# zichunhao/lgn-autoencoder

Measured on AMD Instinct MI355X. Metric: jets/sec fwd+bwd, 30-particle maxdim=2 bs=512, higher is better.
Workload: dtype f64

## Files before the change

### include/lgn_amd.h

```cpp
#ifndef LGN_AMD_H
#define LGN_AMD_H

#include <stddef.h>
#include <stdint.h>

#ifdef __cplusplus
extern "C" {
#endif

#define LGN_AMD_ABI_VERSION 19

int lgn_abi_version(void);
const char* lgn_last_error(void);

int lgn_level_fwd_f64(int B, int N, int C, int CO, int decoder,
                      const double* s_in, const double* v_in, const double* p, const uint8_t* mask,
                      const double* ra, const double* rb, const double* rc,
                      const double* w0, const double* b0, const double* w1, const double* b1,
                      const double* wm0, const double* wm1,
                      double* ag0, double* ag1, double* s_out, double* v_out, void* stream);

int lgn_level_bwd_partial_rows(int B, int N, int decoder, int* rows_mix, int* rows_rad);
int lgn_level_rad_partial_len(int C, int decoder);
int lgn_level_jet_split(int B, int N);

int lgn_level_bwd_f64(int B, int N, int C, int CO, int decoder,
                      const double* s_in, const double* v_in, const double* p, const uint8_t* mask,
                      const double* ra, const double* rb, const double* rc,
                      const double* w0, const double* b0, const double* w1, const double* b1,
                      const double* wm0, const double* wm1, const double* ag0, const double* ag1,
                      const double* g_s_out, const double* g_v_out,
                      double* g_ag, double* g_s_in, double* g_v_in, double* g_p,
                      double* part_mix, double* part_rad, void* stream);

int lgn_cg_product_fwd_f64(int R, int N, int C, int D1, int D2, int DO, int mode, int nnz, const int* row_ptr, const int* col,
                           const double* coef, const double* x1, const double* x2, double* out, void* stream);
int lgn_cg_product_bwd_f64(int R, int N, int C, int D1, int D2, int DO, int mode, int nnz, const int* row_ptr, const int* col,
                           const double* coef, const double* x1, const double* x2, const double* g_out, double* g_x1, double* g_x2,
                           void* stream);

int lgn_reduce_partials_f64(const double* part, int rows, int n, double* out, int accumulate, void* stream);

int lgn_radial_finalize_f64(const double* tot, int C, const double* ra, const double* rb, const double* rc,
                            const double* w0, const double* w1,
                            double* g_a, double* g_b, double* g_c,
                            double* g_w0, double* g_b0, double* g_w1, double* g_b1, void* stream);

#define LGN_ACT_LEAKYRELU 0
#define LGN_ACT_RELU 1
#define LGN_ACT_ELU 2
#define LGN_ACT_SIGMOID 3
#define LGN_ACT_LOGSIGMOID 4
#define LGN_ACT_ATAN 5
#define LGN_ACT_COUNT 6
int lgn_cgmlp_fwd_f64(int M, int C, int H, int nlin, int activation, const double* const* w, const double* const* b,
                      const double* s_in, double* s_out, void* stream);
int lgn_cgmlp_partial_rows(int M, int H);
int lgn_cgmlp_bwd_f64(int M, int C, int H, int nlin, int activation, const double* const* w, const double* const* b,
                      const double* s_in, const double* g_out, double* g_in, double* part, int psize, void* stream);

int lgn_mixreps_fwd_f64(int rows, int Cin, int Cout, int d, const double* w, const double* x, double* y, void* stream);
int lgn_mixreps_partial_rows(int rows);
int lgn_mixreps_bwd_f64(int rows, int Cin, int Cout, int d, const double* w, const double* x, const double* g_y,
                        double* g_x, double* part, void* stream);

int lgn_moments_fwd_f64(int B, int N, int C, int Q, int decoder, const double* X, const double* p, const uint8_t* mask,
                        const double* ra, const double* rb, const double* rc, const double* w0, const double* b0,
                        const double* w1, const double* b1, double* U, void* stream);
long long lgn_moments_scratch_doubles(int B, int N, int C, int decoder);
int lgn_moments_bwd_f64(int B, int N, int C, int Q, int decoder, const double* X, const double* p, const uint8_t* mask,
                        const double* ra, const double* rb, const double* rc, const double* w0, const double* b0,
                        const double* w1, const double* b1, const double* gU, double* gX, double* g_p,
                        double* part_rad, double* scratch, void* stream);

typedef struct lgn_local_tables {
  int n_rows, n_out, n_w;
  int n_terms, n_u, n_x;
  int n_units, static_kind;
  const int *row_ptr, *t_type, *t_a, *t_b;
  const double* t_coef;
  const int *out_dim, *out_nblk, *out_row0, *out_q0, *out_w0;
  const int *u_ptr, *u_row;
  const double* u_coef;
  const int *x_ptr, *x_row, *x_other;
  const double* x_coef;
  int h_out_w0[8];
} lgn_local_tables;

int lgn_local_fwd_f64(int nodes, int C, int CO, int Q, int Qout, const lgn_local_tables* t, const double* X, const double* U,
                      const double* wcat, double* out, void* stream);
int lgn_local_partial_rows(int nodes);
int lgn_local_bwd_f64(int nodes, int C, int CO, int Q, int Qout, const lgn_local_tables* t, const double* X, const double* U,
                      const double* wcat, const double* g_out, double* gU, double* gX, double* part, void* stream);

long long lgn_local_static_packed_doubles(int kind, int C, int CO);
int lgn_local_bwd_static_f64(int kind, int nodes, int C, int CO, const double* XT, const double* UT, const double* wcat,
                             const int* w0, double* wpacked, const double* goT, double* gUT, double* gXT, double* part,
                             double* gpacked, double* g_wcat, void* stream);
int lgn_local_fwd_static_f64(int kind, int nodes, int C, int CO, const double* XT, const double* UT, const double* wcat,
                             const int* w0, double* wpacked, double* outT, double* s_copy, int q_s, void* stream);

typedef struct lgn_net_desc {
  int B, N;
  int n_levels;
  int enc_channels[5];
  int dec_channels[5];
  int tau_s, tau_v;
  int mlp_hidden_mul;
  int mlp_nlin;
  int tau_v_in;
  const lgn_local_tables* enc_tables[4];
  const lgn_local_tables* dec_tables[4];
  int enc_Q[5], enc_qs[5], enc_qv[5];
  int dec_Q[5], dec_qs[5], dec_qv[5];
  int flags;
  int activation;
  int n_in_scalars;
  int latent_pool;
  int dec_N;
  int get_real;
  double jet_loss_scale;
} lgn_net_desc;
#define LGN_REAL_SUM 0
#define LGN_REAL_REAL 1
#define LGN_REAL_IMAG 2
#define LGN_REAL_MEAN 3
#define LGN_REAL_NORM 4
#define LGN_LOSS_CHAMFER 0
#define LGN_LOSS_MSE 1
#define LGN_LOSS_HUNGARIAN 2
typedef struct lgn_loss_desc {
  int kind;
  int abs_coord;
  int polar_coord;
  double scale;
} lgn_loss_desc;
#define LGN_POOL_MIN 0
#define LGN_POOL_MAX 1
#define LGN_POOL_MEAN 2
#define LGN_POOL_MIX 3
#define LGN_POOL(n, avg, o0, o1, o2, o3) ((n) | ((avg) << 3) | ((o0) << 4) | ((o1) << 6) | ((o2) << 8) | ((o3) << 10))
#define LGN_NET_NO_STATIC 1
#define LGN_NET_DEC_PAIRWISE 2
#define LGN_NET_LEVEL_V2 4
#define LGN_NET_MLP_V1 8
#define LGN_NET_MOMENTS_V1 16
#define LGN_NET_BWD_ORDERED 64
#define LGN_NET_DEC_UNFUSED 256
#define LGN_NET_MOMENTS_SPLIT 512
#define LGN_NET_MLP_BWD1 1024
#define LGN_NET_SPLIT_TAIL 128

#define LGN_LDS_LIMIT (160 * 1024)
long long lgn_encoder_end_lds_bytes(int N, int C0, int K, int CL, int Ts, int Tv, int pool);
long long lgn_decoder_end_lds_bytes(int N, int C0, int Tin, int CL);
long long lgn_junction_lds_bytes(int N, int CL, int Ts, int Tv, int pool, int C0);

int lgn_step_param_slots(const lgn_net_desc* d, int decoder);
long long lgn_step_workspace_doubles(const lgn_net_desc* d);
int lgn_step_fwd_bwd_f64(const lgn_net_desc* d, const double* params, double* grads, long long n_params,
                         const int64_t* enc_off, const int64_t* dec_off, const double* p4, const double* target,
                         const uint8_t* mask, const double* in_scalars, double* workspace, long long workspace_doubles,
                         double* recon, double* loss_part, const lgn_loss_desc* loss, int* assignment ,
                         int* status , void* stream);
#define LGN_FINALIZE_SCRATCH 2048
int lgn_step_finalize_f64(double* params, double* grads, long long n_params, const double* loss_part, int n_loss,
                          double l1_lambda, double* adam_m, double* adam_v, long long* step_dev,
                          double lr, double beta1, double beta2, double eps, int do_adam, double* loss_out, void* stream);
int lgn_step_train_f64(const lgn_net_desc* d, double* params, double* grads, long long n_params, const int64_t* enc_off,
                       const int64_t* dec_off, const double* p4, const double* target, const uint8_t* mask, const double* in_scalars,
                       double* workspace, long long workspace_doubles, double* recon, double* loss_part, int n_loss, double l1_lambda,
                       double* adam_m, double* adam_v, long long* step_dev, double lr, double beta1, double beta2, double eps,
                       int do_adam, double* loss_out, const lgn_loss_desc* loss, int* assignment ,
                       int* status , void* stream);

#define LGN_OPT_ADAM 0
#define LGN_OPT_RMSPROP 1
typedef struct {
  int kind;
  double l1_lambda, l2_lambda, lr, eps;
  double beta1, beta2;
  double alpha, momentum;
} lgn_optim_desc;
#define LGN_FINALIZE_OPT_SCRATCH 4096
int lgn_step_finalize_opt_f64(double* params, double* grads, long long n_params, const double* loss_part, int n_loss,
                              const lgn_optim_desc* opt, double* state_m, double* state_v, long long* step_dev, int do_step,
                              double* loss_out, void* stream);
int lgn_step_train_opt_f64(const lgn_net_desc* d, double* params, double* grads, long long n_params, const int64_t* enc_off,
                           const int64_t* dec_off, const double* p4, const double* target, const uint8_t* mask,
                           const double* in_scalars, double* workspace, long long workspace_doubles, double* recon,
                           double* loss_part, int n_loss, const lgn_optim_desc* opt, double* state_m, double* state_v,
                           long long* step_dev, int do_step, double* loss_out, const lgn_loss_desc* loss,
                           int* assignment , int* status , void* stream);

long long lgn_eval_workspace_doubles(const lgn_net_desc* d);
int lgn_step_eval_f64(const lgn_net_desc* d, const double* params, const int64_t* enc_off, const int64_t* dec_off,
                      const double* p4_scaled, const double* p4_target, const uint8_t* mask, const double* in_scalars,
                      double* workspace, long long workspace_doubles, double* recon_real, double* lat_s ,
                      double* lat_v , double* loss_part, double* loss_out, const lgn_loss_desc* loss,
                      int* assignment , int* status , void* stream);

long long lgn_net_workspace_doubles(const lgn_net_desc* d, int decoder, int which);
int lgn_encoder_fwd_f64(const lgn_net_desc* d, const double* params, const int64_t* off, const double* p4, const uint8_t* mask,
                        const double* in_scalars, double* act, long long act_doubles, double* lat_s, double* lat_v, void* stream);
int lgn_encoder_bwd_f64(const lgn_net_desc* d, const double* params, double* grads, long long n_params, const int64_t* off,
                        const double* p4, const uint8_t* mask, const double* in_scalars, const double* act, long long act_doubles,
                        const double* g_lat_s, const double* g_lat_v, double* scratch, long long scratch_doubles, void* stream);
int lgn_decoder_fwd_f64(const lgn_net_desc* d, const double* params, const int64_t* off, const double* lat_v, double* act,
                        long long act_doubles, double* recon, void* stream);
int lgn_decoder_bwd_f64(const lgn_net_desc* d, const double* params, double* grads, long long n_params, const int64_t* off,
                        const double* lat_v, const double* act, long long act_doubles, const double* g_recon, double* g_lat_v,
                        double* scratch, long long scratch_doubles, void* stream);

int lgn_chamfer_f64(int B, int N, int M, const double* x, const double* y, int jet_features, double* loss_part, double* gx, double* gy,
                    void* stream);

#define LGN_ANOMALY_NMAX 192
#define LGN_ANOMALY_NSCORES 21
#define LGN_ANOMALY_ALL 0x1FFFFF
#define LGN_ANOMALY_HUNGARIAN 0x403E0
#define LGN_ANOMALY_NO_HUNGARIAN (LGN_ANOMALY_ALL & ~LGN_ANOMALY_HUNGARIAN)
int lgn_anomaly_scores_f64(const double* recons, const double* target, const double* recons_n, const double* target_n, int B, int N,
                           int score_mask, double* scores, int* col4row , int* status, void* stream);

#define LGN_ROC_TILE 2048
#define LGN_ROC_MAX_COLS 65535
#define LGN_ROC_NONFINITE 1
#define LGN_ROC_SINGLE_CLASS 2
#define LGN_ROC_BAD_LABEL 4
#define LGN_ROC_NAN 8
long long lgn_roc_workspace_bytes(long long M, int K);
int lgn_roc_auc_f64(const double* scores, long long M, int ld, int K, const double* labels, double* fpr, double* tpr,
                    double* thresholds, int* length, double* auc, int* flipped, int* status, void* workspace,
                    long long workspace_bytes, void* stream);

#define LGN_EMD_NMAX 191
#define LGN_EMD_INVALID 1
#define LGN_EMD_EMPTY 2
#define LGN_EMD_ITER 4
#define LGN_EMD_INFEASIBLE 8
long long lgn_emd_workspace_bytes(int B, int N);
long long lgn_emd_lds_bytes(int N);
int lgn_emd_f64(const double* ev0, const double* ev1, int B, int n, int m, double R, double* emd, double* flow ,
                double* dual0 , double* dual1 , int* status, void* work, long long work_bytes, void* stream);
int lgn_emd_relative_f64(const double* recons, const double* target, int B, int N, double* emd, int* status, void* work,
                         long long work_bytes, void* stream);
int lgn_emd_debug_max_augmentations(int* out, int reset);

int lgn_linear_sum_assignment_f64(const double* cost, int B, int n, int* col4row, int* status, void* stream);

int lgn_recon_analysis_f64(const double* target, const double* recons, int B, int N, int abs_coord, int find_match,
                           double* part_polar , double* part_polarrel , double* jet_cart, double* jet_polar,
                           double* jet_rel_err, uint8_t* jet_keep, double* rel_err , int* col4row ,
                           uint8_t* is_padded, int* status, void* stream);

int lgn_match_rel_err_f64(const double* target3, const double* recons3, const double* target_polar, const double* recons_polar,
                          const double* target_polarrel, const double* recons_polarrel, int B, int N, double* rel_err,
                          int* col4row , uint8_t* is_padded, int* status, void* stream);

#define LGN_HIST_MAX_EDGES 1025
#define LGN_HIST_MAX_COLS 16
int lgn_histogram_f64(const double* x, long long rows, int ld, int cols, const double* edges, const int* n_edges , int max_edges,
                      const uint8_t* keep , const double* weights , long long* counts, double* wcounts,
                      int max_bins, void* stream);

#define LGN_STATS_TILE 2048
#define LGN_STATS_MAX_COLS 16
#define LGN_STATS_EMPTY 1
#define LGN_STATS_NONFINITE 2
#define LGN_STAT_MEDIAN 0
#define LGN_STAT_IQR 1
#define LGN_STAT_FIRST_QUARTILE 2
#define LGN_STAT_THIRD_QUARTILE 3
#define LGN_STAT_IDR 4
#define LGN_STAT_MAD 5
#define LGN_STAT_MEAN 6
#define LGN_STAT_MAX 7
#define LGN_STAT_MIN 8
#define LGN_STAT_ABS_MIN 9
#define LGN_STAT_STD_DEV 10
#define LGN_STAT_SKEW 11
#define LGN_STAT_KURTOSIS 12
#define LGN_STAT_FWHM 13
#define LGN_STAT_ABS_MEAN 14
#define LGN_STAT_ABS_MEAN_WITHIN_IQR 15
#define LGN_STAT_ABS_MEAN_WITHIN_IDR 16
#define LGN_STAT_Q10 17
#define LGN_STAT_Q90 18
#define LGN_STATS_COUNT 19
long long lgn_column_stats_workspace_bytes(long long rows, int cols);
int lgn_column_stats_f64(const double* x, long long rows, int ld, int cols, const uint8_t* mask , int mask_keep,
                         double alpha, int num_edges, double* stats ,
                         double* edges , long long* kept ,
                         int* status , void* workspace, long long workspace_bytes, void* stream);

int lgn_hist_fwhm_f64(const long long* counts, int max_bins, const double* edges, int max_edges, const int* n_edges , int cols,
                      double* fwhm , void* stream);

#define LGN_JET_IMAGE_MAX_NPIX 64
#define LGN_JET_IMAGE_PARTS 512
long long lgn_jet_images_workspace_bytes(int B, int npix);
int lgn_jet_images_f64(const double* jets, const double* frame_jets , int B, int N, int mode, int npix, double maxR,
                       int first_n, double* images , double* average, void* workspace, long long workspace_bytes,
                       void* stream);

#define LGN_EQUI_TILE 256
#define LGN_EQUI_MAX_PARTS 64
int lgn_transform_jets_f64(const double* p4, const double* R, const int* perm , const double* scalars , int T,
                           int B, int N, int K, double* out, double* scalars_out , void* stream);
long long lgn_rep_deviation_workspace_bytes(int parts, int T, int B, const int* N , const int* C ,
                                            const int* d );
int lgn_rep_deviation_f64(int parts, int T, int B, const double* const* a , const double* const* b ,
                          const double* const* D , const int* N , const int* C , const int* d ,
                          const int* perm , double* stats , void* workspace, long long workspace_bytes,
                          void* stream);

int lgn_hungarian_mse_f64(int B, int N, const double* x, const double* y, int kind, int abs_coord, int polar_coord, double scale,
                          double* loss_part, double* gx, int* assignment , int* status ,
                          void* stream);
long long lgn_assign_loss_lds_bytes(int N, int C);

#define LGN_NORM_NONE 0
#define LGN_NORM_COMPONENT_MAX 1
#define LGN_NORM_OVERALL_MAX 2
#define LGN_NORM_JET_E 3
int lgn_stage_batch_f64(const double* p4, const uint8_t* labels , const double* scalars , int B, int B_pad, int N,
                        int method, double scale, int jet_features, int K, double* p4_in, double* target, uint8_t* mask,
                        double* in_scalars , double* factor, void* stream);
int lgn_denormalize_f64(const double* x0, const double* x1 , const double* factor, int B, int N, double* out0,
                        double* out1 , void* stream);

#define LGN_EPOCH_MAX_COLLECT 4
#define LGN_EPOCH_BAD_INDEX 1
int lgn_stage_gather_f64(const double* p4, const uint8_t* labels , const double* scalars , long long M,
                         const int* index, long long count, const long long* cursor, int B_pad, int N, int method, double scale,
                         int jet_features, int K, double* p4_in, double* target, uint8_t* mask, double* in_scalars ,
                         double* factor, int* status, void* stream);
int lgn_epoch_collect_f64(const double* loss, double* epoch, long long* cursor, long long count, int B, int n,
                          const double* const* src , double* const* dst , const int* row_doubles , void* stream);
int lgn_epoch_reset(long long* cursor, double* epoch, int* status, void* stream);

#ifdef __cplusplus
}
#endif
#endif
```

### lgn-autoencoder_amd/csrc/api_common.cpp

```cpp
#include <stdarg.h>
#include <stdlib.h>

#include "level.hpp"
#include "../../include/lgn_amd.h"

namespace lgn {
static thread_local char g_err[512] = "";
void set_error(const char* fmt, ...) {
  va_list ap;
  va_start(ap, fmt);
  vsnprintf(g_err, sizeof(g_err), fmt, ap);
  va_end(ap);
}
int level_flags_from_env() {
  auto on = [](const char* name) { const char* e = getenv(name); return e && e[0] == '1'; };
  return (on("LGN_AMD_DEC_PAIRWISE") ? LVL_DEC_PAIRWISE : 0) | (on("LGN_AMD_LEVEL_V2") ? LVL_LEVEL_V2 : 0) |
         (on("LGN_AMD_MOMENTS_V1") ? LVL_MOMENTS_V1 : 0) | (on("LGN_AMD_MLP_V1") ? LVL_MLP_V1 : 0) | (on("LGN_AMD_BWD_ORDERED") ? LVL_BWD_ORDERED : 0) |
         (on("LGN_AMD_MOMENTS_SPLIT") ? LVL_MOMENTS_SPLIT : 0) | (on("LGN_AMD_MLP_BWD1") ? LVL_MLP_BWD1 : 0);
}
static_assert(LVL_DEC_PAIRWISE == LGN_NET_DEC_PAIRWISE && LVL_LEVEL_V2 == LGN_NET_LEVEL_V2 && LVL_MOMENTS_V1 == LGN_NET_MOMENTS_V1 &&
                  LVL_MLP_V1 == LGN_NET_MLP_V1 && LVL_MLP_BWD1 == LGN_NET_MLP_BWD1 &&
                  LVL_BWD_ORDERED == LGN_NET_BWD_ORDERED && LVL_MOMENTS_SPLIT == LGN_NET_MOMENTS_SPLIT, "LVL_* and LGN_NET_* are the same bits");
}

extern "C" {
const char* lgn_last_error(void) { return lgn::g_err; }
int lgn_abi_version(void) { return LGN_AMD_ABI_VERSION; }
}
```

### lgn-autoencoder_amd/csrc/level.hpp

```cpp
#pragma once
#include "common.hpp"

namespace lgn {

constexpr int LVL_DEC_PAIRWISE = 2;
constexpr int LVL_LEVEL_V2 = 4;
constexpr int LVL_MLP_V1 = 8;
constexpr int LVL_MOMENTS_V1 = 16;
constexpr int LVL_MLP_BWD1 = 1024;
constexpr int LVL_MOMENTS_SPLIT = 512;
constexpr int LVL_BWD_ORDERED = 64;
int level_flags_from_env();

template <typename T>
struct LevelArgs {
  int B, N, C, CO;
  const T* s_in;
  const T* v_in;
  const T* p;
  const uint8_t* mask;
  const T *ra, *rb, *rc, *w0, *b0, *w1, *b1;
  const T *wm0, *wm1;
  T* ag0;
  T* ag1;
  T* s_out;
  T* v_out;
  const T* in_w0 = nullptr;
  const T* in_w1 = nullptr;
  T* in_s = nullptr;
  T* in_v = nullptr;
  T* z1 = nullptr;
  size_t z1n = 0;
  T* z2 = nullptr;
  size_t z2n = 0;
  const T* loss_wo1 = nullptr;
  const T* loss_target = nullptr;
  T loss_scale = T(1);
  int loss_real = 0;
  T loss_jscale = T(0);
  T* loss_recon = nullptr;
  T* loss_part = nullptr;
  T* loss_gv = nullptr;
  T* loss_wpart = nullptr;
  int flags = 0;
};

template <typename T>
struct LevelBwdArgs {
  int B, N, C, CO;
  const T *s_in, *v_in, *p;
  const uint8_t* mask;
  const T *ra, *rb, *rc, *w0, *b0, *w1, *b1;
  const T *wm0, *wm1;
  const T *ag0, *ag1;
  const T* g_s_out;
  const T* g_v_out;
  T* g_ag;
  T* g_s_in;
  T* g_v_in;
  T* g_p;
  T* part_mix;
  T* part_rad;
  T* part_in0 = nullptr;
  int flags = 0;
};

__host__ __device__ constexpr int node_stride(int C) { return 10 * C + 4; }

__host__ __device__ constexpr int rad_partial_size(int C, bool dec) {
  return dec ? 2 * C : (2 * 4 * C * NB + 8 * C);
}

inline int level_jet_split(int B, int N) {
  const int groups = (N + 3) / 4;
  int s = 1;
  while (s * 2 <= groups && B * s * 2 <= 512) s *= 2;
  return s;
}

}
```

### lgn-autoencoder_amd/csrc/mlp_chain.hip

```cpp
#include "ops.hpp"

namespace lgn {

typedef double v4d __attribute__((ext_vector_type(4)));
namespace { LGN_STAMP_DECL }
#ifdef LGN_STAMPS
#define DSTAMP(i) do { if (threadIdx.x == 256 && blockIdx.x == 0) g_stamps[i] = clock64(); } while (0)
#else
#define DSTAMP(i) do { } while (0)
#endif
LGN_STAMP_READER(lgn_debug_stamps_mlp_chain)

namespace chain {

__host__ __device__ constexpr int stride2mod4(int x) { return x + ((6 - (x & 3)) & 3); }

__device__ __forceinline__ void lds_barrier() {
  __builtin_amdgcn_sched_barrier(0);
  __builtin_amdgcn_fence(__ATOMIC_RELEASE, "workgroup", "local");
  __builtin_amdgcn_s_barrier();
  __builtin_amdgcn_fence(__ATOMIC_ACQUIRE, "workgroup", "local");
  __builtin_amdgcn_sched_barrier(0);
}
template <int N, int P, class LoadF, class MmaF, class SideF>
__device__ __forceinline__ void mfma_stream(LoadF load, MmaF mma, SideF side) {
  double q[N];
#pragma unroll
  for (int i = 0; i < (P < N ? P : N); ++i) q[i] = load(i);
  __builtin_amdgcn_sched_barrier(0);
#pragma unroll
  for (int i = 0; i < N; ++i) {
    if (i + P < N) q[i + P] = load(i + P);
    mma(i, q[i]);
    side(i);
    __builtin_amdgcn_sched_barrier(0);
  }
}
constexpr int LOOKAHEAD = 9;
template <int N, int T, class F>
__device__ __forceinline__ void deal(int i, F piece) {
  const int j0 = (i * T + N - 1) / N, j1 = ((i + 1) * T + N - 1) / N;
#pragma unroll
  for (int j = j0; j < j1; ++j) piece(j);
}
__device__ __forceinline__ void pin(double& x) { asm volatile("" : "+v"(x)); }

#ifndef LGN_DBG_NOSTAGE
#define LGN_DBG_NOSTAGE 0
#endif
#ifndef LGN_DBG_NOACT
#define LGN_DBG_NOACT 0
#endif
template <bool GEN>
__device__ __forceinline__ double act_t(double x, int act) {
  if (LGN_DBG_NOACT) return x;
  if constexpr (GEN) return act_apply(x, act);
  else return fmax(x, 0.01 * x);
}
template <int H_, int D_, int NST_ = 256>
struct Geo {
  static constexpr int H = H_, D = D_, NH = 6;
  static constexpr int NST = NST_;
  static constexpr int NT = (H + 15) / 16, HP = 16 * NT;
  static constexpr int KSH = H / 4;
  static constexpr int KS0 = (D + 3) / 4;
  static constexpr int S = stride2mod4(HP + 1);
  static constexpr int WSIZE = HP * S;
  static constexpr int SR = NST == 256 ? 66 : 18;
  static constexpr int TSIZE = HP * SR;
  static constexpr int NREG = (HP * 2 * KSH + NST - 1) / NST;
  static_assert(H % 4 == 0 && D <= 16 && D <= H && H <= 96, "chain kernels: H = 12 .. 96 (multiple of 4; the backward: H <= 48), 2C <= 16");
  static constexpr size_t fwd_bytes() { return sizeof(double) * 2 * WSIZE; }
  static constexpr size_t bwd_bytes() { return sizeof(double) * (2 * WSIZE + 4 * TSIZE + (NST == 256 ? 2 * 1024 : 0)); }
  static constexpr int off_w(int l) { return l == 0 ? 0 : (H * D + H) + (l - 1) * (H * H + H); }
  static constexpr int hout(int l) { return l == NH ? D : H; }
  static constexpr int hin(int l) { return l == 0 ? D : H; }
  static constexpr int off_b(int l) { return off_w(l) + hout(l) * hin(l); }
  static constexpr int psize() { return off_b(NH) + D; }
};

template <class G, int L>
struct Img {
  static constexpr int HO = G::hout(L), HI = G::hin(L);
  static constexpr int RP = L == G::NH ? 16 : G::HP;
  static constexpr int CP = L == 0 ? 4 * G::KS0 : 4 * G::KSH;
  static constexpr int CP2 = CP / 2;
  static constexpr int NP = (RP * CP2 + G::NST - 1) / G::NST;
  static_assert(NP <= G::NREG && HI % 2 == 0, "staging registers; rows of an even number of doubles");
};
typedef double v2d __attribute__((ext_vector_type(2)));
template <class G>
struct WRegs {
  v2d v[G::NREG];
  double b;
};
template <class G, int L>
__device__ __forceinline__ void issue_piece(const MlpArgs<double>& a, WRegs<G>& wr, int tid, int j) {
  using I = Img<G, L>;
  if (j < I::NP) {
    const int e = tid + G::NST * j, o = e / I::CP2, k = 2 * (e - o * I::CP2);
    const bool ok = o < I::HO && k < I::HI;
    const v2d x = *reinterpret_cast<const v2d*>(a.w[L] + (ok ? o * I::HI + k : 0));
    wr.v[j] = ok ? x : v2d{0.0, 0.0};
  } else if (j == I::NP) {
    const double bb = a.b[L][tid < I::HO ? tid : 0];
    wr.b = tid < I::HO ? bb : 0.0;
  }
}
template <class G, int L>
__device__ __forceinline__ void commit_piece(double* Wl, const WRegs<G>& wr, int tid, int j) {
  using I = Img<G, L>;
  if (j < I::NP) {
    const int e = tid + G::NST * j, o = e / I::CP2, k = 2 * (e - o * I::CP2);
    if (I::RP * I::CP2 % G::NST == 0 || e < I::RP * I::CP2) *reinterpret_cast<v2d*>(Wl + o * G::S + k) = wr.v[j];
  } else if (j == I::NP) {
    if (tid < I::RP) Wl[tid * G::S + G::HP] = wr.b;
  }
}
template <class G, int L>
__device__ __forceinline__ void issue_image(const MlpArgs<double>& a, WRegs<G>& wr, int tid) {
  using I = Img<G, L>;
#pragma unroll
  for (int i = 0; i < I::NP + 1; ++i) issue_piece<G, L>(a, wr, tid, i);
}
template <class G, int L>
__device__ __forceinline__ void commit_image(double* Wl, const WRegs<G>& wr, int tid) {
  using I = Img<G, L>;
#pragma unroll
  for (int i = 0; i < I::NP + 1; ++i) commit_piece<G, L>(Wl, wr, tid, i);
}
template <class G, bool BWD>
__host__ __device__ constexpr int seq(int q) { return BWD && q > G::NH ? 2 * G::NH - q : q; }
template <class G>
constexpr int stage_pieces() { return 2 * (G::NREG + 1); }
template <class G, bool BWD, int Q>
__device__ __forceinline__ void stage_piece(const MlpArgs<double>& a, double* Wl, WRegs<G>& wrA, WRegs<G>& wrB, int tid, int j) {
  constexpr int LAST = BWD ? 2 * G::NH : G::NH, n1 = Q + 1, n3 = Q + 3;
  WRegs<G>& wr = (n1 & 1) ? wrB : wrA;
  if (j <= G::NREG) {
    if constexpr (n1 <= LAST) commit_piece<G, seq<G, BWD>(n1 <= LAST ? n1 : 0)>(Wl + (n1 & 1) * G::WSIZE, wr, tid, j);
  } else {
    if constexpr (n3 <= LAST) issue_piece<G, seq<G, BWD>(n3 <= LAST ? n3 : 0)>(a, wr, tid, j - G::NREG - 1);
  }
}
template <class G, bool BWD>
__device__ __forceinline__ void stage_prologue(const MlpArgs<double>& a, double* Wl, WRegs<G>& wrA, WRegs<G>& wrB, int tid) {
  issue_image<G, 0>(a, wrA, tid);
  issue_image<G, 1>(a, wrB, tid);
  commit_image<G, 0>(Wl, wrA, tid);
  issue_image<G, 2>(a, wrA, tid);
}

template <class G, int KS, int NTI, bool GEN, int DBG = 0, class ExtF>
__device__ __forceinline__ void layer_fwd(const double* Wc, const v4d (&hin)[NTI], v4d (&hout)[G::NT], int c, int g, int act, ExtF ext) {
  constexpr int S = G::S, NT = G::NT;
  const double* wa = Wc + c * S + g;
  const double* wbias = Wc + g * S + G::HP;
  v4d acc[NT];
#pragma unroll
  for (int r = 0; r < 4; ++r) acc[0][r] = wbias[4 * r * S];
  if (DBG) STAMP(30);
  mfma_stream<KS * NT, LOOKAHEAD>(
      [&](int i) { return wa[16 * (i / KS) * S + 4 * (i % KS)]; },
      [&](int i, double av) {
        const int t = i / KS, ks = i % KS;
        acc[t] = __builtin_amdgcn_mfma_f64_16x16x4f64(av, hin[ks >> 2][ks & 3], acc[t], 0, 0, 0);
      },
      [&](int i) {
        const int t = i / KS, ks = i % KS;
        if (ks == 0 && t + 1 < NT) {
#pragma unroll
          for (int r = 0; r < 4; ++r) acc[t + 1 < NT ? t + 1 : 0][r] = wbias[(16 * (t + 1) + 4 * r) * S];
        }
        constexpr int k1 = KS > 6 ? 5 : KS > 1 ? 1 : 0, k2 = KS > 6 ? 6 : KS > 2 ? 2 : k1;
#pragma unroll
        for (int r = 0; r < 4; ++r)
          if (t > 0 && ks == (r < 2 ? k1 : k2)) {
            double y = act_t<GEN>(acc[t > 0 ? t - 1 : 0][r], act);
            pin(y);
            hout[t > 0 ? t - 1 : 0][r] = y;
          }
        ext(i);
        if (DBG && (i == 0 || i == 1 || i == 2 || i == 11 || i == 12 || i == 23 || i == 34 || i == 35)) STAMP(31 + i);
      });
  if (DBG) STAMP(28);
#pragma unroll
  for (int r = 0; r < 4; ++r) hout[NT - 1][r] = act_t<GEN>(acc[NT - 1][r], act);
  if (DBG) { double z_ = hout[NT - 1][3]; pin(z_); hout[NT - 1][3] = z_; STAMP(29); }
}
template <class G>
__device__ __forceinline__ v4d layer_out(const double* Wc, const v4d (&hin)[G::NT], int c, int g) {
  constexpr int S = G::S;
  const double* wa = Wc + c * S + g;
  v4d acc;
#pragma unroll
  for (int r = 0; r < 4; ++r) acc[r] = Wc[(4 * r + g) * S + G::HP];
  mfma_stream<G::KSH, LOOKAHEAD>([&](int ks) { return wa[4 * ks]; },
                                 [&](int ks, double av) { acc = __builtin_amdgcn_mfma_f64_16x16x4f64(av, hin[ks >> 2][ks & 3], acc, 0, 0, 0); },
                                 [&](int) {});
  return acc;
}
template <class G, int KS, int NTO, int NTG, class FinF, class ExtF>
__device__ __forceinline__ void layer_bwd(const double* Wc, const v4d (&gpre)[NTG], v4d (&gin)[NTO], int c, int g, FinF fin, ExtF ext) {
  constexpr int S = G::S;
  const double* wa = Wc + g * S + c;
#pragma unroll
  for (int u = 0; u < NTO; ++u) gin[u] = v4d{0, 0, 0, 0};
  mfma_stream<KS * NTO, LOOKAHEAD>(
      [&](int i) { return wa[4 * (i % KS) * S + 16 * (i / KS)]; },
      [&](int i, double av) {
        const int u = i / KS, ks = i % KS;
        gin[u] = __builtin_amdgcn_mfma_f64_16x16x4f64(av, gpre[ks >> 2][ks & 3], gin[u], 0, 0, 0);
      },
      [&](int i) {
        const int u = i / KS, ks = i % KS;
        constexpr int k1 = KS > 6 ? 5 : KS > 1 ? 1 : 0, k2 = KS > 6 ? 6 : KS > 2 ? 2 : k1;
#pragma unroll
        for (int r = 0; r < 4; ++r)
          if (u > 0 && ks == (r < 2 ? k1 : k2)) fin(u > 0 ? u - 1 : 0, r);
        ext(i);
      });
}

template <class G>
__device__ __forceinline__ double* saved_ptr(const MlpArgs<double>& a, int wave, int lane) {
  return a.h_saved + ((size_t)blockIdx.x * 4 + wave) * (G::NH * G::NT * 256) + lane * 4;
}
template <class G>
constexpr int saved_pieces() { return 2 * G::NT; }
template <class G, int NTI>
__device__ __forceinline__ void save_piece(double* hs, int l, const v4d (&h)[NTI], int j) {
  const v2d v = {h[j >> 1][2 * (j & 1)], h[j >> 1][2 * (j & 1) + 1]};
  __builtin_nontemporal_store(v, reinterpret_cast<v2d*>(hs + (l * G::NT + (j >> 1)) * 256 + 2 * (j & 1)));
}
template <class G>
__device__ __forceinline__ void load_piece(const double* hs, int l, v4d (&h)[G::NT], int j) {
  const v2d v = __builtin_nontemporal_load(reinterpret_cast<const v2d*>(hs + (l * G::NT + (j >> 1)) * 256 + 2 * (j & 1)));
  h[j >> 1][2 * (j & 1)] = v[0];
  h[j >> 1][2 * (j & 1) + 1] = v[1];
}

template <class G>
__device__ __forceinline__ void load_x(const MlpArgs<double>& a, int row, int g, v4d (&xb)[1]) {
  const bool rok = row < a.M;
#pragma unroll
  for (int r = 0; r < 4; ++r) {
    const int f = 4 * r + g;
    const bool ok = r < G::KS0 && rok && f < G::D;
    const double x = a.s_in[ok ? (size_t)(f & 1) * a.M * a.C + (size_t)row * a.C + (f >> 1) : 0];
    xb[0][r] = ok ? x : 0.0;
  }
}

template <int H, int D, bool GEN, bool SAVE, bool TWO = false>
__global__ __launch_bounds__(TWO ? 512 : 256) void mlp_chain_fwd_kernel(MlpArgs<double> a) {
  using G = Geo<H, D>;
  const int tid = threadIdx.x, lane = tid & 63, wave = __builtin_amdgcn_readfirstlane(tid >> 6);
  const int c = lane & 15, g = lane >> 4;
  const int row = blockIdx.x * 64 + wave * 16 + c;
  extern __shared__ __align__(16) unsigned char smem_raw[];
  double* Wl = reinterpret_cast<double*>(smem_raw);
  WRegs<G> wrA, wrB;
  STAMP(0);
  STAMP_LIFE_BEGIN();
  if constexpr (TWO) {
    if (wave >= 4) {
      const int st = tid - 256;
      stage_prologue<G, false>(a, Wl, wrA, wrB, st);
      lds_barrier();
#define LGN_STAGE_STEP(Q)                                                                                            \
  _Pragma("unroll") for (int j = 0; j < stage_pieces<G>(); ++j) stage_piece<G, false, Q>(a, Wl, wrA, wrB, st, j);    \
  lds_barrier();
      LGN_STAGE_STEP(0) LGN_STAGE_STEP(1) LGN_STAGE_STEP(2) LGN_STAGE_STEP(3) LGN_STAGE_STEP(4) LGN_STAGE_STEP(5)
#undef LGN_STAGE_STEP
      return;
    }
  }
  v4d xb[1];
  load_x<G>(a, row, g, xb);
  if constexpr (!TWO) stage_prologue<G, false>(a, Wl, wrA, wrB, tid);
  lds_barrier();
  STAMP(1);
  v4d h0[G::NT], h1[G::NT];
  double* hs = SAVE ? saved_ptr<G>(a, wave, lane) : nullptr;
#define LGN_CHAIN_STEP(Q, HIN, HOUT, KS, NTI)                                                                        \
  layer_fwd<G, KS, NTI, GEN, (Q == 3)>(Wl + (Q & 1) * G::WSIZE, HIN, HOUT, c, g, a.act, [&](int i) {               \
    if (!TWO && !LGN_DBG_NOSTAGE) deal<KS * G::NT, stage_pieces<G>()>(i, [&](int j) { stage_piece<G, false, Q>(a, Wl, wrA, wrB, tid, j); });      \
    if (SAVE && Q > 0) deal<KS * G::NT, 2 * NTI>(i, [&](int j) { save_piece<G>(hs, Q - 1, HIN, j); });              \
  });                                                                                                                \
  lds_barrier();                                                                                                     \
  STAMP(2 + Q);
  LGN_CHAIN_STEP(0, xb, h0, G::KS0, 1)
  LGN_CHAIN_STEP(1, h0, h1, G::KSH, G::NT)
  LGN_CHAIN_STEP(2, h1, h0, G::KSH, G::NT)
  LGN_CHAIN_STEP(3, h0, h1, G::KSH, G::NT)
  LGN_CHAIN_STEP(4, h1, h0, G::KSH, G::NT)
  LGN_CHAIN_STEP(5, h0, h1, G::KSH, G::NT)
#undef LGN_CHAIN_STEP
  if (SAVE) {
#pragma unroll
    for (int j = 0; j < saved_pieces<G>(); ++j) save_piece<G>(hs, G::NH - 1, h1, j);
  }
  const v4d y = layer_out<G>(Wl + (G::NH & 1) * G::WSIZE, h1, c, g);
#pragma unroll
  for (int r = 0; r < 4; ++r) {
    const int o = 4 * r + g;
    if (o < D && row < a.M) a.s_out[mlp_out_index(a, o & 1, row, o >> 1)] = y[r];
  }
  STAMP(8);
  STAMP_LIFE_END();
}

template <class G, int NTI>
__device__ __forceinline__ void publish_piece(double* T, const v4d (&v)[NTI], int wave, int c, int g, int j) {
  T[(4 * j + g) * G::SR + 16 * wave + c] = v[j >> 2][j & 3];
}
template <class G, int L, int NU, class SideF>
__device__ __forceinline__ void dw_unit(const double* Gt, const double* Xt, double* part, int t, int u0, int c, int g, SideF side) {
  constexpr int SR = G::SR, HO = G::hout(L), HI = G::hin(L), N = 16 * NU, P = 6;
  const double* ga = Gt + (16 * t + c) * SR + g;
  const double* xb = Xt + (16 * u0 + c) * SR + g;
  double* pW = part + G::off_w(L);
  v4d acc[NU];
#pragma unroll
  for (int u = 0; u < NU; ++u) acc[u] = v4d{0, 0, 0, 0};
  double dbs = 0.0, qa[16], qx[N];
  auto load = [&](int i) {
    qx[i] = xb[16 * (i >> 4) * SR + 4 * (i & 15)];
    if (i < 16) qa[i] = ga[4 * i];
  };
  auto store = [&](int u, int r) {
    const int o = 16 * t + 4 * r + g, k = 16 * (u0 + u) + c;
    if (o < HO && k < HI) __builtin_nontemporal_store(acc[u][r], &pW[o * HI + k]);
  };
#pragma unroll
  for (int i = 0; i < P; ++i) load(i);
  __builtin_amdgcn_sched_barrier(0);
#pragma unroll
  for (int i = 0; i < N; ++i) {
    const int u = i >> 4, sk = i & 15;
    if (i + P < N) load(i + P);
    acc[u] = __builtin_amdgcn_mfma_f64_16x16x4f64(qa[sk], qx[i], acc[u], 0, 0, 0);
    if (u > 0 && sk >= 1 && sk <= 4) store(u > 0 ? u - 1 : 0, sk - 1);
    side(i);
    __builtin_amdgcn_sched_barrier(0);
  }
#pragma unroll
  for (int r = 0; r < 4; ++r) store(NU - 1, r);
  if (u0 == 0) {
    double d4[4] = {0.0, 0.0, 0.0, 0.0};
#pragma unroll
    for (int sk = 0; sk < 16; ++sk) d4[sk & 3] += qa[sk];
    dbs = (d4[0] + d4[1]) + (d4[2] + d4[3]);
    dbs += shfl_xor(dbs, 16);
    dbs += shfl_xor(dbs, 32);
    if (g == 0 && 16 * t + c < HO) __builtin_nontemporal_store(dbs, &part[G::off_b(L) + 16 * t + c]);
  }
}
template <class G, int L, class SideF>
__device__ __forceinline__ bool dw_layer(const double* Gt, const double* Xt, double* part, int wave, int c, int g, SideF side) {
  if (L == G::NH) {
    if (wave < G::NT) { dw_unit<G, L, 1>(Gt, Xt, part, 0, wave, c, g, side); return true; }
  } else if (L == 0) {
    if (wave < G::NT) { dw_unit<G, L, 1>(Gt, Xt, part, wave, 0, c, g, side); return true; }
  } else {
    const int t = (wave + L) & 3;
    if (t < G::NT) { dw_unit<G, L, G::NT>(Gt, Xt, part, t, 0, c, g, side); return true; }
  }
  return false;
}

template <int H, int D, bool GEN, bool SAVE>
__global__ __launch_bounds__(256) void mlp_chain_bwd_kernel(MlpArgs<double> a) {
  using G = Geo<H, D>;
  constexpr int NT = G::NT, NH = G::NH;
  const int tid = threadIdx.x, lane = tid & 63, wave = __builtin_amdgcn_readfirstlane(tid >> 6);
  const int c = lane & 15, g = lane >> 4;
  const int row = blockIdx.x * 64 + wave * 16 + c;
  extern __shared__ __align__(16) unsigned char smem_raw[];
  double* Wl = reinterpret_cast<double*>(smem_raw);
  double* Gt = Wl + 2 * G::WSIZE;
  double* Xt = Gt + 2 * G::TSIZE;
  double* part = a.part + (size_t)blockIdx.x * a.psize;
  WRegs<G> wrA, wrB;
  STAMP(10);
  v4d xb[1];
  load_x<G>(a, row, g, xb);
  v4d gout[1];
#pragma unroll
  for (int r = 0; r < 4; ++r) {
    const int o = 4 * r + g;
    const bool ok = o < D && row < a.M;
    const double x = a.g_out[ok ? mlp_out_index(a, o & 1, row, o >> 1) : 0];
    gout[0][r] = ok ? x : 0.0;
  }
  v4d h[NH][NT];
  const double* hs = SAVE ? saved_ptr<G>(a, wave, lane) : nullptr;
  if constexpr (SAVE) {
    issue_image<G, NH>(a, wrA, tid);
    issue_image<G, NH - 1>(a, wrB, tid);
#pragma unroll
    for (int j = 0; j < saved_pieces<G>(); ++j) load_piece<G>(hs, NH - 1, h[NH - 1], j);
#pragma unroll
    for (int j = 0; j < saved_pieces<G>(); ++j) load_piece<G>(hs, NH - 2, h[NH - 2], j);
    commit_image<G, NH>(Wl, wrA, tid);
    issue_image<G, NH - 2>(a, wrA, tid);
    lds_barrier();
    STAMP(11);
  } else {
    stage_prologue<G, true>(a, Wl, wrA, wrB, tid);
    lds_barrier();
    STAMP(11);
#define LGN_CHAIN_STEP(Q, HIN, KS, NTI)                                                                              \
  layer_fwd<G, KS, NTI, GEN>(Wl + (Q & 1) * G::WSIZE, HIN, h[Q], c, g, a.act, [&](int i) {                          \
    deal<KS * NT, stage_pieces<G>()>(i, [&](int j) { stage_piece<G, true, Q>(a, Wl, wrA, wrB, tid, j); });          \
  });                                                                                                                \
  lds_barrier();                                                                                                     \
  STAMP(12 + Q);
    LGN_CHAIN_STEP(0, xb, G::KS0, 1)
    LGN_CHAIN_STEP(1, h[0], G::KSH, NT)
    LGN_CHAIN_STEP(2, h[1], G::KSH, NT)
    LGN_CHAIN_STEP(3, h[2], G::KSH, NT)
    LGN_CHAIN_STEP(4, h[3], G::KSH, NT)
    LGN_CHAIN_STEP(5, h[4], G::KSH, NT)
#undef LGN_CHAIN_STEP
  }
  v4d gpA[NT], gpB[NT], gin[NT];
  {
    constexpr int NI = G::KS0 * NT, NSV = SAVE && NH >= 3 ? saved_pieces<G>() : 0, NPC = 4 + 4 * NT + stage_pieces<G>() + NSV;
    auto fin = [&](int u, int r) {
      double y = gin[u][r] * act_slope_t<GEN>(h[NH - 1][u][r], a.act);
      pin(y);
      gpA[u][r] = y;
    };
    layer_bwd<G, G::KS0, NT, 1>(Wl + 0 * G::WSIZE, gout, gin, c, g, fin, [&](int i) {
      deal<NI, NPC>(i, [&](int j) {
        if (j < 4) publish_piece<G, 1>(Gt, gout, wave, c, g, j);
        else if (j < 4 + 4 * NT) publish_piece<G, NT>(Xt, h[NH - 1], wave, c, g, j - 4);
        else if (j < 4 + 4 * NT + stage_pieces<G>()) stage_piece<G, true, NH>(a, Wl, wrA, wrB, tid, j - 4 - 4 * NT);
        else if constexpr (NSV > 0) load_piece<G>(hs, NH - 3, h[NH >= 3 ? NH - 3 : 0], j - 4 - 4 * NT - stage_pieces<G>());
      });
    });
#pragma unroll
    for (int r = 0; r < 4; ++r) fin(NT - 1, r);
    lds_barrier();
    STAMP(18);
  }
#define LGN_CHAIN_BSTEP(L, GP, GN)                                                                                   \
  {                                                                                                                  \
    constexpr int q_ = 2 * NH - (L), NI = G::KSH * NT, NSV = SAVE && (L) >= 3 ? saved_pieces<G>() : 0,               \
                  NPC = 8 * NT + stage_pieces<G>() + NSV;                                                            \
    auto fin = [&](int u, int r) {                                                                                   \
      double y = gin[u][r] * act_slope_t<GEN>(h[(L) - 1][u][r], a.act);                                              \
      pin(y);                                                                                                        \
      GN[u][r] = y;                                                                                                  \
    };                                                                                                               \
    layer_bwd<G, G::KSH, NT, NT>(Wl + (q_ & 1) * G::WSIZE, GP, gin, c, g, fin, [&](int i) {                          \
      deal<NI, NPC>(i, [&](int j) {                                                                                  \
        if (j < 4 * NT) publish_piece<G, NT>(Gt + ((L) & 1) * G::TSIZE, GP, wave, c, g, j);                          \
        else if (j < 8 * NT) publish_piece<G, NT>(Xt + ((L) & 1) * G::TSIZE, h[(L) - 1], wave, c, g, j - 4 * NT);    \
        else if (j < 8 * NT + stage_pieces<G>()) stage_piece<G, true, q_>(a, Wl, wrA, wrB, tid, j - 8 * NT);         \
        else if constexpr (NSV > 0) load_piece<G>(hs, (L) - 3, h[(L) >= 3 ? (L) - 3 : 0], j - 8 * NT - stage_pieces<G>()); \
      });                                                                                                            \
    });                                                                                                              \
    auto tail = [&](int i) {                                                                                         \
      if (i == 1) { fin(NT - 1, 0); fin(NT - 1, 1); }                                                                \
      if (i == 2) { fin(NT - 1, 2); fin(NT - 1, 3); }                                                                \
    };                                                                                                               \
    if (!dw_layer<G, (L) + 1>(Gt + (((L) + 1) & 1) * G::TSIZE, Xt + (((L) + 1) & 1) * G::TSIZE, part, wave, c, g, tail)) {   \
      tail(1);                                                                                                       \
      tail(2);                                                                                                       \
    }                                                                                                                \
    lds_barrier();                                                                                                   \
    STAMP(12 + q_);                                                                                                  \
  }
  LGN_CHAIN_BSTEP(5, gpA, gpB)
  LGN_CHAIN_BSTEP(4, gpB, gpA)
  LGN_CHAIN_BSTEP(3, gpA, gpB)
  LGN_CHAIN_BSTEP(2, gpB, gpA)
  LGN_CHAIN_BSTEP(1, gpA, gpB)
#undef LGN_CHAIN_BSTEP
  {
    v4d gx[1];
    layer_bwd<G, G::KSH, 1, NT>(Wl + 0 * G::WSIZE, gpB, gx, c, g, [&](int, int) {}, [&](int i) {
      deal<G::KSH, 4 * NT + 4>(i, [&](int j) {
        if (j < 4 * NT) publish_piece<G, NT>(Gt, gpB, wave, c, g, j);
        else publish_piece<G, 1>(Xt, xb, wave, c, g, j - 4 * NT);
      });
    });
    auto tail = [&](int i) {
      if (i >= 1 && i <= 4) {
        const int f = 4 * (i - 1) + g;
        if (f < D && row < a.M) a.g_in[mlp_out_index(a, f & 1, row, f >> 1)] = gx[0][i - 1];
      }
    };
    if (!dw_layer<G, 1>(Gt + G::TSIZE, Xt + G::TSIZE, part, wave, c, g, tail)) {
#pragma unroll
      for (int i = 1; i <= 4; ++i) tail(i);
    }
    lds_barrier();
    STAMP(25);
  }
  dw_layer<G, 0>(Gt, Xt, part, wave, c, g, [&](int) {});
  STAMP(26);
}

template <class G, int L, class SideF>
__device__ __forceinline__ void dw_hidden3(const double* Gt, const double* Xt, double* part, double* qs, int w, int lane, int c, int g, SideF side) {
  static_assert(G::NT == 3 && L >= 1 && L < G::NH, "hidden layers of three tiles");
  constexpr int SR = G::SR, H = G::H, N = 36, P = 6;
  const int i0 = 2 * w, i1 = 2 * w + 1;
  const int t0 = i0 / 3, u0 = i0 - 3 * t0, t1 = i1 / 3, u1 = i1 - 3 * t1;
  const double* ga0 = Gt + (16 * t0 + c) * SR + g;
  const double* xb0 = Xt + (16 * u0 + c) * SR + g;
  const double* ga1 = Gt + (16 * t1 + c) * SR + g;
  const double* xb1 = Xt + (16 * u1 + c) * SR + g;
  const double* ga2 = Gt + (32 + c) * SR + g + 16 * w;
  const double* xb2 = Xt + (32 + c) * SR + g + 16 * w;
  double* pW = part + G::off_w(L);
  v4d acc0 = {0, 0, 0, 0}, acc1 = {0, 0, 0, 0}, acc2 = {0, 0, 0, 0};
  double qa[N], qx[N];
  auto load = [&](int i) {
    if (i < 16) { qa[i] = ga0[4 * i]; qx[i] = xb0[4 * i]; }
    else if (i < 32) { qa[i] = ga1[4 * (i - 16)]; qx[i] = xb1[4 * (i - 16)]; }
    else { qa[i] = ga2[4 * (i - 32)]; qx[i] = xb2[4 * (i - 32)]; }
  };
  auto store = [&](const v4d& acc, int t, int u, int r) {
    const int o = 16 * t + 4 * r + g, k = 16 * u + c;
    if (o < H && k < H) __builtin_nontemporal_store(acc[r], &pW[o * H + k]);
  };
#pragma unroll
  for (int i = 0; i < P; ++i) load(i);
  __builtin_amdgcn_sched_barrier(0);
#pragma unroll
  for (int i = 0; i < N; ++i) {
    if (i + P < N) load(i + P);
    if (i < 16) acc0 = __builtin_amdgcn_mfma_f64_16x16x4f64(qa[i], qx[i], acc0, 0, 0, 0);
    else if (i < 32) acc1 = __builtin_amdgcn_mfma_f64_16x16x4f64(qa[i], qx[i], acc1, 0, 0, 0);
    else acc2 = __builtin_amdgcn_mfma_f64_16x16x4f64(qa[i], qx[i], acc2, 0, 0, 0);
    if (i >= 17 && i <= 20) store(acc0, t0, u0, i - 17);
    if (i >= 33) store(acc1, t1, u1, i - 33);
    side(i);
    __builtin_amdgcn_sched_barrier(0);
  }
  store(acc1, t1, u1, 3);
#pragma unroll
  for (int r = 0; r < 4; ++r) qs[(w * 4 + r) * 64 + lane] = acc2[r];
  if (w != 1) {
    double d4[4] = {0.0, 0.0, 0.0, 0.0};
#pragma unroll
    for (int sk = 0; sk < 16; ++sk) d4[sk & 3] += qa[sk];
    double dbs = (d4[0] + d4[1]) + (d4[2] + d4[3]);
    dbs += shfl_xor(dbs, 16);
    dbs += shfl_xor(dbs, 32);
    if (g == 0 && 16 * t0 + c < H) __builtin_nontemporal_store(dbs, &part[G::off_b(L) + 16 * t0 + c]);
  }
}
template <class G, int L>
__device__ __forceinline__ void dw_quarter_sum(const double* qs, double* part, int lane, int c, int g) {
  constexpr int H = G::H;
  double* pW = part + G::off_w(L);
#pragma unroll
  for (int r = 0; r < 4; ++r) {
    const double v = (qs[(0 * 4 + r) * 64 + lane] + qs[(1 * 4 + r) * 64 + lane]) + (qs[(2 * 4 + r) * 64 + lane] + qs[(3 * 4 + r) * 64 + lane]);
    const int o = 32 + 4 * r + g, k = 32 + c;
    if (o < H && k < H) __builtin_nontemporal_store(v, &pW[o * H + k]);
  }
}

template <int H, int D, bool GEN>
__global__ __launch_bounds__(512) void mlp_chain_bwd2_kernel(MlpArgs<double> a) {
  using G = Geo<H, D>;
  constexpr int NT = G::NT, NH = G::NH;
  const int lane = threadIdx.x & 63, wave = __builtin_amdgcn_readfirstlane((int)threadIdx.x >> 6);
  const int w4 = wave & 3;
  const int c = lane & 15, g = lane >> 4;
  extern __shared__ __align__(16) unsigned char smem_raw[];
  double* Wl = reinterpret_cast<double*>(smem_raw);
  double* Gt = Wl + 2 * G::WSIZE;
  double* Xt = Gt + 2 * G::TSIZE;
  STAMP(10);
  if (wave >= 4) {
    __builtin_amdgcn_s_setprio(2);
    const int tid = (int)threadIdx.x - 256;
    double* part = a.part + (size_t)blockIdx.x * a.psize;
    WRegs<G> wrA, wrB;
    stage_prologue<G, true>(a, Wl, wrA, wrB, tid);
    lds_barrier();
#define LGN_STAGE_ALL(Q)                                                                                             \
  _Pragma("unroll") for (int j = 0; j < stage_pieces<G>(); ++j) stage_piece<G, true, Q>(a, Wl, wrA, wrB, tid, j);
#define LGN_STAGE_STEP(Q) LGN_STAGE_ALL(Q) lds_barrier();
    LGN_STAGE_STEP(0) LGN_STAGE_STEP(1) LGN_STAGE_STEP(2) LGN_STAGE_STEP(3) LGN_STAGE_STEP(4) LGN_STAGE_STEP(5)
    LGN_STAGE_STEP(6)
    constexpr bool EVEN = NT == 3;
    double* qs = Xt + 2 * G::TSIZE;
#define LGN_DW_STEP(L)                                                                                               \
  {                                                                                                                  \
    constexpr int q_ = 2 * NH - (L), NS = stage_pieces<G>(), L1 = (L) + 1;                                           \
    constexpr bool HID = EVEN && L1 >= 1 && L1 < NH;                                                                 \
    constexpr int NI = HID ? 36 : (L1 == NH || L1 == 0) ? 16 : 16 * NT;                                              \
    auto side = [&](int i) { deal<NI, NS>(i, [&](int j) { stage_piece<G, true, q_>(a, Wl, wrA, wrB, tid, j); }); };  \
    if constexpr (EVEN && L1 + 1 >= 1 && L1 + 1 < NH) {                                                              \
      if (w4 == 1) dw_quarter_sum<G, (L1 + 1 < NH ? L1 + 1 : 1)>(qs + ((L1 + 1) & 1) * 1024, part, lane, c, g);     \
    }                                                                                                                \
    if constexpr (HID) {                                                                                             \
      dw_hidden3<G, (HID ? L1 : 1)>(Gt + (L1 & 1) * G::TSIZE, Xt + (L1 & 1) * G::TSIZE, part, qs + (L1 & 1) * 1024, w4, lane, c, g, side); \
    } else if (!dw_layer<G, L1>(Gt + (L1 & 1) * G::TSIZE, Xt + (L1 & 1) * G::TSIZE, part, w4, c, g, side)) {         \
      LGN_STAGE_ALL(q_)                                                                                              \
    }                                                                                                                \
    DSTAMP(44 + (L));                                                                                                \
    lds_barrier();                                                                                                   \
  }
    LGN_DW_STEP(5) LGN_DW_STEP(4) LGN_DW_STEP(3) LGN_DW_STEP(2) LGN_DW_STEP(1) LGN_DW_STEP(0)
#undef LGN_DW_STEP
#undef LGN_STAGE_STEP
#undef LGN_STAGE_ALL
    if constexpr (EVEN && NH >= 2) {
      if (w4 == 1) dw_quarter_sum<G, 1>(qs + 1024, part, lane, c, g);
    }
    dw_layer<G, 0>(Gt, Xt, part, w4, c, g, [&](int) {});
    return;
  }
  const int row = blockIdx.x * 64 + wave * 16 + c;
  v4d xb[1];
  load_x<G>(a, row, g, xb);
  v4d gout[1];
#pragma unroll
  for (int r = 0; r < 4; ++r) {
    const int o = 4 * r + g;
    const bool ok = o < D && row < a.M;
    const double x = a.g_out[ok ? mlp_out_index(a, o & 1, row, o >> 1) : 0];
    gout[0][r] = ok ? x : 0.0;
  }
  v4d h[NH][NT];
  lds_barrier();
  STAMP(11);
#define LGN_CHAIN_STEP(Q, HIN, KS, NTI)                                                                              \
  layer_fwd<G, KS, NTI, GEN>(Wl + (Q & 1) * G::WSIZE, HIN, h[Q], c, g, a.act, [&](int) {});                          \
  lds_barrier();                                                                                                     \
  STAMP(12 + Q);
  LGN_CHAIN_STEP(0, xb, G::KS0, 1)
  LGN_CHAIN_STEP(1, h[0], G::KSH, NT)
  LGN_CHAIN_STEP(2, h[1], G::KSH, NT)
  LGN_CHAIN_STEP(3, h[2], G::KSH, NT)
  LGN_CHAIN_STEP(4, h[3], G::KSH, NT)
  LGN_CHAIN_STEP(5, h[4], G::KSH, NT)
#undef LGN_CHAIN_STEP
  v4d gpA[NT], gpB[NT], gin[NT];
  {
    constexpr int NI = G::KS0 * NT, NPC = 4 + 4 * NT;
    auto fin = [&](int u, int r) {
      double y = gin[u][r] * act_slope_t<GEN>(h[NH - 1][u][r], a.act);
      pin(y);
      gpA[u][r] = y;
    };
    layer_bwd<G, G::KS0, NT, 1>(Wl + 0 * G::WSIZE, gout, gin, c, g, fin, [&](int i) {
      deal<NI, NPC>(i, [&](int j) {
        if (j < 4) publish_piece<G, 1>(Gt, gout, wave, c, g, j);
        else publish_piece<G, NT>(Xt, h[NH - 1], wave, c, g, j - 4);
      });
    });
#pragma unroll
    for (int r = 0; r < 4; ++r) fin(NT - 1, r);
    lds_barrier();
    STAMP(18);
  }
#define LGN_CHAIN_BSTEP(L, GP, GN)                                                                                   \
  {                                                                                                                  \
    constexpr int q_ = 2 * NH - (L), NI = G::KSH * NT, NPC = 8 * NT;                                                 \
    auto fin = [&](int u, int r) {                                                                                   \
      double y = gin[u][r] * act_slope_t<GEN>(h[(L) - 1][u][r], a.act);                                              \
      pin(y);                                                                                                        \
      GN[u][r] = y;                                                                                                  \
    };                                                                                                               \
    layer_bwd<G, G::KSH, NT, NT>(Wl + (q_ & 1) * G::WSIZE, GP, gin, c, g, fin, [&](int i) {                          \
      deal<NI, NPC>(i, [&](int j) {                                                                                  \
        if (j < 4 * NT) publish_piece<G, NT>(Gt + ((L) & 1) * G::TSIZE, GP, wave, c, g, j);                          \
        else publish_piece<G, NT>(Xt + ((L) & 1) * G::TSIZE, h[(L) - 1], wave, c, g, j - 4 * NT);                    \
      });                                                                                                            \
    });                                                                                                              \
    STAMP(56 + (L));                                                                                                 \
    _Pragma("unroll") for (int r = 0; r < 4; ++r) fin(NT - 1, r);                                                    \
    STAMP(50 + (L));                                                                                                 \
    lds_barrier();                                                                                                   \
    STAMP(12 + q_);                                                                                                  \
  }
  LGN_CHAIN_BSTEP(5, gpA, gpB)
  LGN_CHAIN_BSTEP(4, gpB, gpA)
  LGN_CHAIN_BSTEP(3, gpA, gpB)
  LGN_CHAIN_BSTEP(2, gpB, gpA)
  LGN_CHAIN_BSTEP(1, gpA, gpB)
#undef LGN_CHAIN_BSTEP
  {
    v4d gx[1];
    layer_bwd<G, G::KSH, 1, NT>(Wl + 0 * G::WSIZE, gpB, gx, c, g, [&](int, int) {}, [&](int i) {
      deal<G::KSH, 4 * NT + 4>(i, [&](int j) {
        if (j < 4 * NT) publish_piece<G, NT>(Gt, gpB, wave, c, g, j);
        else publish_piece<G, 1>(Xt, xb, wave, c, g, j - 4 * NT);
      });
    });
#pragma unroll
    for (int r = 0; r < 4; ++r) {
      const int f = 4 * r + g;
      if (f < D && row < a.M) a.g_in[mlp_out_index(a, f & 1, row, f >> 1)] = gx[0][r];
    }
    lds_barrier();
    STAMP(25);
  }
}

template <class G>
__device__ __forceinline__ double* saved_ptr16(const MlpArgs<double>& a, int lane) {
  return a.h_saved + (size_t)blockIdx.x * (G::NH * G::NT * 256) + lane * 4;
}
template <int H, int D, bool GEN, bool SAVE>
__global__ __launch_bounds__(192) void mlp_chain_fwd16_kernel(MlpArgs<double> a) {
  using G = Geo<H, D, 128>;
  const int tid = threadIdx.x, lane = tid & 63, wave = __builtin_amdgcn_readfirstlane(tid >> 6);
  const int c = lane & 15, g = lane >> 4;
  extern __shared__ __align__(16) unsigned char smem_raw[];
  double* Wl = reinterpret_cast<double*>(smem_raw);
  if (wave >= 1) {
    const int st = tid - 64;
    WRegs<G> wrA, wrB;
    stage_prologue<G, false>(a, Wl, wrA, wrB, st);
    lds_barrier();
#define LGN_STAGE_STEP(Q)                                                                                            \
  _Pragma("unroll") for (int j = 0; j < stage_pieces<G>(); ++j) stage_piece<G, false, Q>(a, Wl, wrA, wrB, st, j);    \
  lds_barrier();
    LGN_STAGE_STEP(0) LGN_STAGE_STEP(1) LGN_STAGE_STEP(2) LGN_STAGE_STEP(3) LGN_STAGE_STEP(4) LGN_STAGE_STEP(5)
#undef LGN_STAGE_STEP
    return;
  }
  const int row = blockIdx.x * 16 + c;
  v4d xb[1];
  load_x<G>(a, row, g, xb);
  lds_barrier();
  v4d h0[G::NT], h1[G::NT];
  double* hs = SAVE ? saved_ptr16<G>(a, lane) : nullptr;
#define LGN_CHAIN_STEP(Q, HIN, HOUT, KS, NTI)                                                                        \
  layer_fwd<G, KS, NTI, GEN>(Wl + (Q & 1) * G::WSIZE, HIN, HOUT, c, g, a.act, [&](int i) {                          \
    if (SAVE && Q > 0) deal<KS * G::NT, 2 * NTI>(i, [&](int j) { save_piece<G>(hs, Q - 1, HIN, j); });              \
  });                                                                                                                \
  lds_barrier();
  LGN_CHAIN_STEP(0, xb, h0, G::KS0, 1)
  LGN_CHAIN_STEP(1, h0, h1, G::KSH, G::NT)
  LGN_CHAIN_STEP(2, h1, h0, G::KSH, G::NT)
  LGN_CHAIN_STEP(3, h0, h1, G::KSH, G::NT)
  LGN_CHAIN_STEP(4, h1, h0, G::KSH, G::NT)
  LGN_CHAIN_STEP(5, h0, h1, G::KSH, G::NT)
#undef LGN_CHAIN_STEP
  if (SAVE) {
#pragma unroll
    for (int j = 0; j < saved_pieces<G>(); ++j) save_piece<G>(hs, G::NH - 1, h1, j);
  }
  const v4d y = layer_out<G>(Wl + (G::NH & 1) * G::WSIZE, h1, c, g);
#pragma unroll
  for (int r = 0; r < 4; ++r) {
    const int o = 4 * r + g;
    if (o < D && row < a.M) a.s_out[mlp_out_index(a, o & 1, row, o >> 1)] = y[r];
  }
}

template <class G, int L>
__device__ __forceinline__ void dw16(const double* Gt, const double* Xt, double* part, int c, int g) {
  constexpr int SR = G::SR, HO = G::hout(L), HI = G::hin(L);
  constexpr int NTO = L == G::NH ? 1 : G::NT, NTI = L == 0 ? 1 : G::NT, NTL = NTO * NTI;
  double* pW = part + G::off_w(L);
  double qa[NTO][4], qx[NTI][4];
#pragma unroll
  for (int t = 0; t < NTO; ++t)
#pragma unroll
    for (int sk = 0; sk < 4; ++sk) qa[t][sk] = Gt[(16 * t + c) * SR + g + 4 * sk];
#pragma unroll
  for (int u = 0; u < NTI; ++u)
#pragma unroll
    for (int sk = 0; sk < 4; ++sk) qx[u][sk] = Xt[(16 * u + c) * SR + g + 4 * sk];
  __builtin_amdgcn_sched_barrier(0);
  v4d acc[NTL];
  auto store = [&](int tile, int r) {
    const int t = tile / NTI, u = tile - t * NTI, o = 16 * t + 4 * r + g, k = 16 * u + c;
    if (o < HO && k < HI) __builtin_nontemporal_store(acc[tile][r], &pW[o * HI + k]);
  };
#pragma unroll
  for (int i = 0; i < 4 * NTL; ++i) {
    const int tile = i >> 2, sk = i & 3, t = tile / NTI, u = tile - t * NTI;
    if (sk == 0) acc[tile] = v4d{0, 0, 0, 0};
    acc[tile] = __builtin_amdgcn_mfma_f64_16x16x4f64(qa[t][sk], qx[u][sk], acc[tile], 0, 0, 0);
    if (tile > 0) store(tile > 0 ? tile - 1 : 0, sk);
    __builtin_amdgcn_sched_barrier(0);
  }
#pragma unroll
  for (int r = 0; r < 4; ++r) store(NTL - 1, r);
#pragma unroll
  for (int t = 0; t < NTO; ++t) {
    double dbs = (qa[t][0] + qa[t][1]) + (qa[t][2] + qa[t][3]);
    dbs += shfl_xor(dbs, 16);
    dbs += shfl_xor(dbs, 32);
    if (g == 0 && 16 * t + c < HO) __builtin_nontemporal_store(dbs, &part[G::off_b(L) + 16 * t + c]);
  }
}

template <int H, int D, bool GEN, bool SAVE>
__global__ __launch_bounds__(256) void mlp_chain_bwd16_kernel(MlpArgs<double> a) {
  using G = Geo<H, D, 128>;
  constexpr int NT = G::NT, NH = G::NH;
  const int lane = threadIdx.x & 63, wave = __builtin_amdgcn_readfirstlane((int)threadIdx.x >> 6);
  const int c = lane & 15, g = lane >> 4;
  extern __shared__ __align__(16) unsigned char smem_raw[];
  double* Wl = reinterpret_cast<double*>(smem_raw);
  double* Gt = Wl + 2 * G::WSIZE;
  double* Xt = Gt + 2 * G::TSIZE;
  if (wave >= 2) {
    const int st = (int)threadIdx.x - 128;
    WRegs<G> wrA, wrB;
#define LGN_STAGE_STEP(Q)                                                                                            \
  _Pragma("unroll") for (int j = 0; j < stage_pieces<G>(); ++j) stage_piece<G, true, Q>(a, Wl, wrA, wrB, st, j);     \
  lds_barrier();
    if constexpr (SAVE) {
      issue_image<G, NH>(a, wrA, st);
      issue_image<G, NH - 1>(a, wrB, st);
      commit_image<G, NH>(Wl, wrA, st);
      issue_image<G, NH - 2>(a, wrA, st);
      lds_barrier();
    } else {
      stage_prologue<G, true>(a, Wl, wrA, wrB, st);
      lds_barrier();
      LGN_STAGE_STEP(0) LGN_STAGE_STEP(1) LGN_STAGE_STEP(2) LGN_STAGE_STEP(3) LGN_STAGE_STEP(4) LGN_STAGE_STEP(5)
    }
    LGN_STAGE_STEP(6) LGN_STAGE_STEP(7) LGN_STAGE_STEP(8) LGN_STAGE_STEP(9) LGN_STAGE_STEP(10) LGN_STAGE_STEP(11) LGN_STAGE_STEP(12)
#undef LGN_STAGE_STEP
    return;
  }
  if (wave == 1) {
    double* part = a.part + (size_t)blockIdx.x * a.psize;
    lds_barrier();
    if constexpr (!SAVE) {
#pragma unroll
      for (int q = 0; q < 6; ++q) lds_barrier();
    }
    lds_barrier();
    dw16<G, 6>(Gt + 0 * G::TSIZE, Xt + 0 * G::TSIZE, part, c, g);  lds_barrier();
    dw16<G, 5>(Gt + 1 * G::TSIZE, Xt + 1 * G::TSIZE, part, c, g);  lds_barrier();
    dw16<G, 4>(Gt + 0 * G::TSIZE, Xt + 0 * G::TSIZE, part, c, g);  lds_barrier();
    dw16<G, 3>(Gt + 1 * G::TSIZE, Xt + 1 * G::TSIZE, part, c, g);  lds_barrier();
    dw16<G, 2>(Gt + 0 * G::TSIZE, Xt + 0 * G::TSIZE, part, c, g);  lds_barrier();
    dw16<G, 1>(Gt + 1 * G::TSIZE, Xt + 1 * G::TSIZE, part, c, g);  lds_barrier();
    dw16<G, 0>(Gt, Xt, part, c, g);
    return;
  }
  const int row = blockIdx.x * 16 + c;
  v4d xb[1];
  load_x<G>(a, row, g, xb);
  v4d gout[1];
#pragma unroll
  for (int r = 0; r < 4; ++r) {
    const int o = 4 * r + g;
    const bool ok = o < D && row < a.M;
    const double x = a.g_out[ok ? mlp_out_index(a, o & 1, row, o >> 1) : 0];
    gout[0][r] = ok ? x : 0.0;
  }
  v4d h[NH][NT];
  const double* hs = SAVE ? saved_ptr16<G>(a, lane) : nullptr;
  if constexpr (SAVE) {
#pragma unroll
    for (int j = 0; j < saved_pieces<G>(); ++j) load_piece<G>(hs, NH - 1, h[NH - 1], j);
#pragma unroll
    for (int j = 0; j < saved_pieces<G>(); ++j) load_piece<G>(hs, NH - 2, h[NH - 2], j);
    lds_barrier();
  } else {
    lds_barrier();
#define LGN_CHAIN_STEP(Q, HIN, KS, NTI)                                                                              \
  layer_fwd<G, KS, NTI, GEN>(Wl + (Q & 1) * G::WSIZE, HIN, h[Q], c, g, a.act, [&](int) {});                          \
  lds_barrier();
    LGN_CHAIN_STEP(0, xb, G::KS0, 1)
    LGN_CHAIN_STEP(1, h[0], G::KSH, NT)
    LGN_CHAIN_STEP(2, h[1], G::KSH, NT)
    LGN_CHAIN_STEP(3, h[2], G::KSH, NT)
    LGN_CHAIN_STEP(4, h[3], G::KSH, NT)
    LGN_CHAIN_STEP(5, h[4], G::KSH, NT)
#undef LGN_CHAIN_STEP
  }
  v4d gpA[NT], gpB[NT], gin[NT];
  {
    constexpr int NI = G::KS0 * NT, NSV = SAVE && NH >= 3 ? saved_pieces<G>() : 0, NPC = 4 + 4 * NT + NSV;
    auto fin = [&](int u, int r) {
      double y = gin[u][r] * act_slope_t<GEN>(h[NH - 1][u][r], a.act);
      pin(y);
      gpA[u][r] = y;
    };
    layer_bwd<G, G::KS0, NT, 1>(Wl + 0 * G::WSIZE, gout, gin, c, g, fin, [&](int i) {
      deal<NI, NPC>(i, [&](int j) {
        if (j < 4) publish_piece<G, 1>(Gt, gout, 0, c, g, j);
        else if (j < 4 + 4 * NT) publish_piece<G, NT>(Xt, h[NH - 1], 0, c, g, j - 4);
        else if constexpr (NSV > 0) load_piece<G>(hs, NH - 3, h[NH >= 3 ? NH - 3 : 0], j - 4 - 4 * NT);
      });
    });
#pragma unroll
    for (int r = 0; r < 4; ++r) fin(NT - 1, r);
    lds_barrier();
  }
#define LGN_CHAIN_BSTEP(L, GP, GN)                                                                                   \
  {                                                                                                                  \
    constexpr int q_ = 2 * NH - (L), NI = G::KSH * NT, NSV = SAVE && (L) >= 3 ? saved_pieces<G>() : 0, NPC = 8 * NT + NSV; \
    auto fin = [&](int u, int r) {                                                                                   \
      double y = gin[u][r] * act_slope_t<GEN>(h[(L) - 1][u][r], a.act);                                              \
      pin(y);                                                                                                        \
      GN[u][r] = y;                                                                                                  \
    };                                                                                                               \
    layer_bwd<G, G::KSH, NT, NT>(Wl + (q_ & 1) * G::WSIZE, GP, gin, c, g, fin, [&](int i) {                          \
      deal<NI, NPC>(i, [&](int j) {                                                                                  \
        if (j < 4 * NT) publish_piece<G, NT>(Gt + ((L) & 1) * G::TSIZE, GP, 0, c, g, j);                             \
        else if (j < 8 * NT) publish_piece<G, NT>(Xt + ((L) & 1) * G::TSIZE, h[(L) - 1], 0, c, g, j - 4 * NT);       \
        else if constexpr (NSV > 0) load_piece<G>(hs, (L) - 3, h[(L) >= 3 ? (L) - 3 : 0], j - 8 * NT);               \
      });                                                                                                            \
    });                                                                                                              \
    _Pragma("unroll") for (int r = 0; r < 4; ++r) fin(NT - 1, r);                                                    \
    lds_barrier();                                                                                                   \
  }
  LGN_CHAIN_BSTEP(5, gpA, gpB)
  LGN_CHAIN_BSTEP(4, gpB, gpA)
  LGN_CHAIN_BSTEP(3, gpA, gpB)
  LGN_CHAIN_BSTEP(2, gpB, gpA)
  LGN_CHAIN_BSTEP(1, gpA, gpB)
#undef LGN_CHAIN_BSTEP
  {
    v4d gx[1];
    layer_bwd<G, G::KSH, 1, NT>(Wl + 0 * G::WSIZE, gpB, gx, c, g, [&](int, int) {}, [&](int i) {
      deal<G::KSH, 4 * NT + 4>(i, [&](int j) {
        if (j < 4 * NT) publish_piece<G, NT>(Gt, gpB, 0, c, g, j);
        else publish_piece<G, 1>(Xt, xb, 0, c, g, j - 4 * NT);
      });
    });
#pragma unroll
    for (int r = 0; r < 4; ++r) {
      const int f = 4 * r + g;
      if (f < D && row < a.M) a.g_in[mlp_out_index(a, f & 1, row, f >> 1)] = gx[0][r];
    }
    lds_barrier();
  }
}

template <class G, int KS>
__device__ __forceinline__ void split_operands(const double* T, const double (&own)[4], int t, int c, int g, double (&hb)[KS]) {
  const int nown = KS - 4 * t < 4 ? KS - 4 * t : 4;
#pragma unroll
  for (int i = 0; i < KS; ++i) {
    int ks = 4 * t + i;
    if (ks >= KS) ks -= KS;
    const double v = T[(4 * ks + g) * G::SR + c];
    hb[i] = (i < 4 && i < nown) ? own[i < 4 ? i : 0] : v;
  }
}
template <int H, int D, bool GEN, bool SAVE>
__global__ __launch_bounds__(320) void mlp_chain_fwd16s_kernel(MlpArgs<double> a) {
  using G = Geo<H, D, 128>;
  static_assert(G::NT == 3, "three chain waves");
  constexpr int S = G::S, SR = G::SR, NH = G::NH, KSH = G::KSH, KS0 = G::KS0, HP = G::HP;
  const int tid = threadIdx.x, lane = tid & 63, wave = __builtin_amdgcn_readfirstlane(tid >> 6);
  const int c = lane & 15, g = lane >> 4;
  extern __shared__ __align__(16) unsigned char smem_raw[];
  double* Wl = reinterpret_cast<double*>(smem_raw);
  double* At = Wl + 2 * G::WSIZE;
  if (wave >= 3) {
    const int st = tid - 192;
    WRegs<G> wrA, wrB;
    stage_prologue<G, false>(a, Wl, wrA, wrB, st);
    lds_barrier();
#define LGN_STAGE_STEP(Q)                                                                                            \
  _Pragma("unroll") for (int j = 0; j < stage_pieces<G>(); ++j) stage_piece<G, false, Q>(a, Wl, wrA, wrB, st, j);    \
  lds_barrier();
    LGN_STAGE_STEP(0) LGN_STAGE_STEP(1) LGN_STAGE_STEP(2) LGN_STAGE_STEP(3) LGN_STAGE_STEP(4) LGN_STAGE_STEP(5)
#undef LGN_STAGE_STEP
    return;
  }
  const int t = wave, row = blockIdx.x * 16 + c;
  v4d xb[1];
  load_x<G>(a, row, g, xb);
  double* hs = SAVE ? saved_ptr16<G>(a, lane) + t * 256 : nullptr;
  lds_barrier();
  double own[4];
  auto finish = [&](int q, v4d& acc) {
    double* T = At + (q & 1) * G::TSIZE;
#pragma unroll
    for (int r = 0; r < 4; ++r) {
      own[r] = act_t<GEN>(acc[r], a.act);
      T[(16 * t + 4 * r + g) * SR + c] = own[r];
    }
    if (SAVE) {
#pragma unroll
      for (int hf = 0; hf < 2; ++hf)
        *reinterpret_cast<v2d*>(hs + q * G::NT * 256 + 2 * hf) = v2d{own[2 * hf], own[2 * hf + 1]};
    }
  };
  {
    const double* Wc = Wl;
    const double* wa = Wc + (16 * t + c) * S + g;
    v4d acc;
#pragma unroll
    for (int r = 0; r < 4; ++r) acc[r] = Wc[(16 * t + 4 * r + g) * S + HP];
    mfma_stream<KS0, LOOKAHEAD>([&](int i) { return wa[4 * i]; },
                                [&](int i, double av) { acc = __builtin_amdgcn_mfma_f64_16x16x4f64(av, xb[0][i], acc, 0, 0, 0); }, [&](int) {});
    finish(0, acc);
    lds_barrier();
  }
#pragma unroll
  for (int q = 1; q < NH; ++q) {
    const double* Wc = Wl + (q & 1) * G::WSIZE;
    const double* wa = Wc + (16 * t + c) * S + g;
    double hb[KSH];
    split_operands<G, KSH>(At + ((q - 1) & 1) * G::TSIZE, own, t, c, g, hb);
    v4d acc;
#pragma unroll
    for (int r = 0; r < 4; ++r) acc[r] = Wc[(16 * t + 4 * r + g) * S + HP];
    mfma_stream<KSH, LOOKAHEAD>([&](int i) { int ks = 4 * t + i; if (ks >= KSH) ks -= KSH; return wa[4 * ks]; },
                                [&](int i, double av) { acc = __builtin_amdgcn_mfma_f64_16x16x4f64(av, hb[i], acc, 0, 0, 0); }, [&](int) {});
    finish(q, acc);
    lds_barrier();
  }
  if (t != 0) return;
  {
    const double* Wc = Wl + (NH & 1) * G::WSIZE;
    const double* wa = Wc + c * S + g;
    double hb[KSH];
    split_operands<G, KSH>(At + ((NH - 1) & 1) * G::TSIZE, own, 0, c, g, hb);
    v4d y;
#pragma unroll
    for (int r = 0; r < 4; ++r) y[r] = Wc[(4 * r + g) * S + HP];
    mfma_stream<KSH, LOOKAHEAD>([&](int i) { return wa[4 * i]; },
                                [&](int i, double av) { y = __builtin_amdgcn_mfma_f64_16x16x4f64(av, hb[i], y, 0, 0, 0); }, [&](int) {});
#pragma unroll
    for (int r = 0; r < 4; ++r) {
      const int o = 4 * r + g;
      if (o < D && row < a.M) a.s_out[mlp_out_index(a, o & 1, row, o >> 1)] = y[r];
    }
  }
}

template <class G, int L, int NW = 4>
__device__ __forceinline__ void dw16_part(const double* Gt, const double* Xt, double* part, int w, int c, int g) {
  constexpr int SR = G::SR, HO = G::hout(L), HI = G::hin(L);
  constexpr int NTO = L == G::NH ? 1 : G::NT, NTI = L == 0 ? 1 : G::NT, NTL = NTO * NTI;
  double* pW = part + G::off_w(L);
  double qa[NTO][4], qx[NTI][4];
#pragma unroll
  for (int t = 0; t < NTO; ++t)
#pragma unroll
    for (int sk = 0; sk < 4; ++sk) qa[t][sk] = Gt[(16 * t + c) * SR + g + 4 * sk];
#pragma unroll
  for (int u = 0; u < NTI; ++u)
#pragma unroll
    for (int sk = 0; sk < 4; ++sk) qx[u][sk] = Xt[(16 * u + c) * SR + g + 4 * sk];
  __builtin_amdgcn_sched_barrier(0);
  v4d acc[NTL];
  auto store = [&](int tile) {
    const int t = tile / NTI, u = tile - t * NTI;
#pragma unroll
    for (int r = 0; r < 4; ++r) {
      const int o = 16 * t + 4 * r + g, k = 16 * u + c;
      if (o < HO && k < HI) __builtin_nontemporal_store(acc[tile][r], &pW[o * HI + k]);
    }
  };
#pragma unroll
  for (int tile = 0; tile < NTL; ++tile) {
    if (tile % NW == w) {
      const int t = tile / NTI, u = tile - t * NTI;
      acc[tile] = v4d{0, 0, 0, 0};
#pragma unroll
      for (int sk = 0; sk < 4; ++sk) acc[tile] = __builtin_amdgcn_mfma_f64_16x16x4f64(qa[t][sk], qx[u][sk], acc[tile], 0, 0, 0);
      if (tile >= NW) store(tile >= NW ? tile - NW : 0);
      __builtin_amdgcn_sched_barrier(0);
    }
  }
#pragma unroll
  for (int tile = (NTL > NW ? NTL - NW : 0); tile < NTL; ++tile)
    if (tile % NW == w) store(tile);
  if (w == 0) {
#pragma unroll
    for (int t = 0; t < NTO; ++t) {
      double dbs = (qa[t][0] + qa[t][1]) + (qa[t][2] + qa[t][3]);
      dbs += shfl_xor(dbs, 16);
      dbs += shfl_xor(dbs, 32);
      if (g == 0 && 16 * t + c < HO) __builtin_nontemporal_store(dbs, &part[G::off_b(L) + 16 * t + c]);
    }
  }
}

template <int H, int D, bool GEN>
__global__ __launch_bounds__(576) void mlp_chain_bwd16s_kernel(MlpArgs<double> a) {
  using G = Geo<H, D, 128>;
  static_assert(G::NT == 3, "three chain waves");
  constexpr int S = G::S, SR = G::SR, NT = G::NT, NH = G::NH, KSH = G::KSH, KS0 = G::KS0;
  const int lane = threadIdx.x & 63, wave = __builtin_amdgcn_readfirstlane((int)threadIdx.x >> 6);
  const int c = lane & 15, g = lane >> 4;
  extern __shared__ __align__(16) unsigned char smem_raw[];
  double* Wl = reinterpret_cast<double*>(smem_raw);
  double* Gt = Wl + 2 * G::WSIZE;
  double* Xt = Gt + 2 * G::TSIZE;
  if (wave >= 7) {
    const int st = (int)threadIdx.x - 448;
    WRegs<G> wrA, wrB;
    issue_image<G, NH>(a, wrA, st);
    issue_image<G, NH - 1>(a, wrB, st);
    commit_image<G, NH>(Wl, wrA, st);
    issue_image<G, NH - 2>(a, wrA, st);
    lds_barrier();
#define LGN_STAGE_STEP(Q)                                                                                            \
  _Pragma("unroll") for (int j = 0; j < stage_pieces<G>(); ++j) stage_piece<G, true, Q>(a, Wl, wrA, wrB, st, j);     \
  lds_barrier();
    LGN_STAGE_STEP(6) LGN_STAGE_STEP(7) LGN_STAGE_STEP(8) LGN_STAGE_STEP(9) LGN_STAGE_STEP(10) LGN_STAGE_STEP(11)
#undef LGN_STAGE_STEP
    return;
  }
  if (wave >= 3) {
    const int w = wave - 3;
    double* part = a.part + (size_t)blockIdx.x * a.psize;
    lds_barrier();
    dw16_part<G, 6>(Gt + 0 * G::TSIZE, Xt + 0 * G::TSIZE, part, w, c, g);  lds_barrier();
    dw16_part<G, 5>(Gt + 1 * G::TSIZE, Xt + 1 * G::TSIZE, part, w, c, g);  lds_barrier();
    dw16_part<G, 4>(Gt + 0 * G::TSIZE, Xt + 0 * G::TSIZE, part, w, c, g);  lds_barrier();
    dw16_part<G, 3>(Gt + 1 * G::TSIZE, Xt + 1 * G::TSIZE, part, w, c, g);  lds_barrier();
    dw16_part<G, 2>(Gt + 0 * G::TSIZE, Xt + 0 * G::TSIZE, part, w, c, g);  lds_barrier();
    dw16_part<G, 1>(Gt + 1 * G::TSIZE, Xt + 1 * G::TSIZE, part, w, c, g);  lds_barrier();
    dw16_part<G, 0>(Gt, Xt, part, w, c, g);
    return;
  }
  const int u = wave, row = blockIdx.x * 16 + c;
  STAMP(10);
  const double* hs = saved_ptr16<G>(a, lane) + u * 256;
  double hown[NH][4];
#pragma unroll
  for (int l = 0; l < NH; ++l)
#pragma unroll
    for (int hf = 0; hf < 2; ++hf) {
      const v2d v = *reinterpret_cast<const v2d*>(hs + l * NT * 256 + 2 * hf);
      hown[l][2 * hf] = v[0];
      hown[l][2 * hf + 1] = v[1];
    }
  v4d xb[1], gout[1];
  load_x<G>(a, row, g, xb);
#pragma unroll
  for (int r = 0; r < 4; ++r) {
    const int o = 4 * r + g;
    const bool ok = o < D && row < a.M;
    const double x = a.g_out[ok ? mlp_out_index(a, o & 1, row, o >> 1) : 0];
    gout[0][r] = ok ? x : 0.0;
  }
  auto publish = [&](double* T, const double (&v)[4]) {
#pragma unroll
    for (int r = 0; r < 4; ++r) T[(16 * u + 4 * r + g) * SR + c] = v[r];
  };
  auto publish1 = [&](double* T, const v4d& v) {
    if (u == 0) {
#pragma unroll
      for (int r = 0; r < 4; ++r) T[(4 * r + g) * SR + c] = v[r];
    }
  };
  STAMP(27);
  publish1(Gt, gout[0]);
  publish(Xt, hown[NH - 1]);
  lds_barrier();
  STAMP(11);
  double gp[4];
  {
    const double* Wc = Wl;
    const double* wa = Wc + g * S + 16 * u + c;
    v4d gin = {0, 0, 0, 0};
    mfma_stream<KS0, LOOKAHEAD>([&](int i) { return wa[4 * i * S]; },
                                [&](int i, double av) { gin = __builtin_amdgcn_mfma_f64_16x16x4f64(av, gout[0][i], gin, 0, 0, 0); }, [&](int) {});
#pragma unroll
    for (int r = 0; r < 4; ++r) gp[r] = gin[r] * act_slope_t<GEN>(hown[NH - 1][r], a.act);
    publish(Gt + G::TSIZE, gp);
    publish(Xt + G::TSIZE, hown[NH - 2]);
    lds_barrier();
    STAMP(12);
  }
#pragma unroll
  for (int L = NH - 1; L >= 1; --L) {
    const double* Wc = Wl + (L & 1) * G::WSIZE;
    const double* wa = Wc + g * S + 16 * u + c;
    double hb[KSH];
    split_operands<G, KSH>(Gt + (L & 1) * G::TSIZE, gp, u, c, g, hb);
    v4d gin = {0, 0, 0, 0};
    mfma_stream<KSH, LOOKAHEAD>([&](int i) { int ks = 4 * u + i; if (ks >= KSH) ks -= KSH; return wa[4 * ks * S]; },
                                [&](int i, double av) { gin = __builtin_amdgcn_mfma_f64_16x16x4f64(av, hb[i], gin, 0, 0, 0); }, [&](int) {});
#pragma unroll
    for (int r = 0; r < 4; ++r) gp[r] = gin[r] * act_slope_t<GEN>(hown[L - 1][r], a.act);
    publish(Gt + ((L - 1) & 1) * G::TSIZE, gp);
    if (L >= 2) publish(Xt + ((L - 1) & 1) * G::TSIZE, hown[L >= 2 ? L - 2 : 0]);
    else publish1(Xt, xb[0]);
    STAMP(20 + L);
    lds_barrier();
    STAMP(12 + NH - L);
  }
  if (u != 0) return;
  {
    const double* Wc = Wl;
    const double* wa = Wc + g * S + c;
    double hb[KSH];
    split_operands<G, KSH>(Gt, gp, 0, c, g, hb);
    v4d gx = {0, 0, 0, 0};
    mfma_stream<KSH, LOOKAHEAD>([&](int i) { return wa[4 * i * S]; },
                                [&](int i, double av) { gx = __builtin_amdgcn_mfma_f64_16x16x4f64(av, hb[i], gx, 0, 0, 0); }, [&](int) {});
#pragma unroll
    for (int r = 0; r < 4; ++r) {
      const int f = 4 * r + g;
      if (f < D && row < a.M) a.g_in[mlp_out_index(a, f & 1, row, f >> 1)] = gx[r];
    }
    STAMP(19);
  }
}

template <int H, int D>
static int launch16s(const MlpArgs<double>& a, bool backward, hipStream_t stream) {
  using G = Geo<H, D, 128>;
  const int nblk = cdiv(a.M, 16);
  const size_t smem = sizeof(double) * (2 * G::WSIZE + (backward ? 4 : 2) * G::TSIZE);
  if (backward) LGN_CHECK_ARG(a.psize == G::psize(), "cgmlp: psize %d, expected %d", a.psize, G::psize());
  LGN_CHECK_ARG(!a.h_saved || a.h_rows >= nblk * 16, "cgmlp: the saved-activation buffer has %d rows per layer, %d rows need %d",
                a.h_rows, a.M, nblk * 16);
  void (*kern)(MlpArgs<double>);
  if (backward) kern = a.act == 0 ? mlp_chain_bwd16s_kernel<H, D, false> : mlp_chain_bwd16s_kernel<H, D, true>;
  else kern = a.h_saved ? (a.act == 0 ? mlp_chain_fwd16s_kernel<H, D, false, true> : mlp_chain_fwd16s_kernel<H, D, true, true>)
                        : (a.act == 0 ? mlp_chain_fwd16s_kernel<H, D, false, false> : mlp_chain_fwd16s_kernel<H, D, true, false>);
  if (smem > 64 * 1024) (void)hipFuncSetAttribute(reinterpret_cast<const void*>(kern), hipFuncAttributeMaxDynamicSharedMemorySize, (int)smem);
  hipLaunchKernelGGL(kern, dim3(nblk), dim3(backward ? 576 : 320), smem, stream, a);
  LGN_CHECK_LAUNCH();
  return 0;
}

template <int H, int D>
static int launch16(const MlpArgs<double>& a, bool backward, hipStream_t stream) {
  using G = Geo<H, D, 128>;
  const int nblk = cdiv(a.M, 16);
  const size_t smem = backward ? G::bwd_bytes() : G::fwd_bytes();
  if (backward) LGN_CHECK_ARG(a.psize == G::psize(), "cgmlp: psize %d, expected %d", a.psize, G::psize());
  LGN_CHECK_ARG(!a.h_saved || a.h_rows >= nblk * 16, "cgmlp: the saved-activation buffer has %d rows per layer, %d rows need %d",
                a.h_rows, a.M, nblk * 16);
  void (*kern)(MlpArgs<double>);
  if (backward) kern = a.h_saved ? (a.act == 0 ? mlp_chain_bwd16_kernel<H, D, false, true> : mlp_chain_bwd16_kernel<H, D, true, true>)
                                 : (a.act == 0 ? mlp_chain_bwd16_kernel<H, D, false, false> : mlp_chain_bwd16_kernel<H, D, true, false>);
  else kern = a.h_saved ? (a.act == 0 ? mlp_chain_fwd16_kernel<H, D, false, true> : mlp_chain_fwd16_kernel<H, D, true, true>)
                        : (a.act == 0 ? mlp_chain_fwd16_kernel<H, D, false, false> : mlp_chain_fwd16_kernel<H, D, true, false>);
  if (smem > 64 * 1024) (void)hipFuncSetAttribute(reinterpret_cast<const void*>(kern), hipFuncAttributeMaxDynamicSharedMemorySize, (int)smem);
  hipLaunchKernelGGL(kern, dim3(nblk), dim3(backward ? 256 : 192), smem, stream, a);
  LGN_CHECK_LAUNCH();
  return 0;
}

template <int H, int D>
static int launch_fwd(const MlpArgs<double>& a, hipStream_t stream) {
  using G = Geo<H, D>;
  static_assert(G::fwd_bytes() <= 160 * 1024, "LDS budget");
  const bool two = !(a.flags & LVL_MLP_BWD1);
  auto kern = two ? (a.act == 0 ? mlp_chain_fwd_kernel<H, D, false, false, true> : mlp_chain_fwd_kernel<H, D, true, false, true>)
                  : (a.act == 0 ? mlp_chain_fwd_kernel<H, D, false, false> : mlp_chain_fwd_kernel<H, D, true, false>);
  (void)hipFuncSetAttribute(reinterpret_cast<const void*>(kern), hipFuncAttributeMaxDynamicSharedMemorySize, (int)G::fwd_bytes());
  hipLaunchKernelGGL(kern, dim3(cdiv(a.M, 64)), dim3(two ? 512 : 256), G::fwd_bytes(), stream, a);
  LGN_CHECK_LAUNCH();
  return 0;
}

template <int H, int D>
static int launch(const MlpArgs<double>& a, bool backward, hipStream_t stream) {
  using G = Geo<H, D>;
  const int nblk = cdiv(a.M, 64);
  const size_t smem = backward ? G::bwd_bytes() : G::fwd_bytes();
  static_assert(G::bwd_bytes() <= 160 * 1024, "LDS budget");
  if (backward) LGN_CHECK_ARG(a.psize == G::psize(), "cgmlp: psize %d, expected %d", a.psize, G::psize());
  LGN_CHECK_ARG(!a.h_saved || a.h_rows >= nblk * 64, "cgmlp: the saved-activation buffer has %d rows per layer, %d rows need %d",
                a.h_rows, a.M, nblk * 64);
  if (backward && !a.h_saved && !(a.flags & LVL_MLP_BWD1)) {
    auto k2 = a.act == 0 ? mlp_chain_bwd2_kernel<H, D, false> : mlp_chain_bwd2_kernel<H, D, true>;
    if (smem > 64 * 1024) (void)hipFuncSetAttribute(reinterpret_cast<const void*>(k2), hipFuncAttributeMaxDynamicSharedMemorySize, (int)smem);
    hipLaunchKernelGGL(k2, dim3(nblk), dim3(512), smem, stream, a);
    LGN_CHECK_LAUNCH();
    return 0;
  }
  if (!backward && !a.h_saved && !(a.flags & LVL_MLP_BWD1)) {
    auto k2 = a.act == 0 ? mlp_chain_fwd_kernel<H, D, false, false, true> : mlp_chain_fwd_kernel<H, D, true, false, true>;
    if (smem > 64 * 1024) (void)hipFuncSetAttribute(reinterpret_cast<const void*>(k2), hipFuncAttributeMaxDynamicSharedMemorySize, (int)smem);
    hipLaunchKernelGGL(k2, dim3(nblk), dim3(512), smem, stream, a);
    LGN_CHECK_LAUNCH();
    return 0;
  }
  auto kern = a.h_saved ? (a.act == 0 ? (backward ? mlp_chain_bwd_kernel<H, D, false, true> : mlp_chain_fwd_kernel<H, D, false, true>)
                                      : (backward ? mlp_chain_bwd_kernel<H, D, true, true> : mlp_chain_fwd_kernel<H, D, true, true>))
                        : (a.act == 0 ? (backward ? mlp_chain_bwd_kernel<H, D, false, false> : mlp_chain_fwd_kernel<H, D, false, false>)
                                      : (backward ? mlp_chain_bwd_kernel<H, D, true, false> : mlp_chain_fwd_kernel<H, D, true, false>));
  if (smem > 64 * 1024) (void)hipFuncSetAttribute(reinterpret_cast<const void*>(kern), hipFuncAttributeMaxDynamicSharedMemorySize, (int)smem);
  hipLaunchKernelGGL(kern, dim3(nblk), dim3(256), smem, stream, a);
  LGN_CHECK_LAUNCH();
  return 0;
}

}

int mlp_chain_dispatch(const MlpArgs<double>& a, bool backward, hipStream_t stream) {
  if ((a.flags & LVL_MLP_V1) || a.nlin != 7) return -2;
  if (mlp_rows_per_workgroup(a.M, a.H) != 64) {
    if (!(a.flags & LVL_MLP_BWD1) && (!backward || a.h_saved)) {
      if (a.H == 48 && a.C == 4) return chain::launch16s<48, 8>(a, backward, stream);
      if (a.H == 36 && a.C == 3) return chain::launch16s<36, 6>(a, backward, stream);
    }
    if (a.H == 48 && a.C == 4) return chain::launch16<48, 8>(a, backward, stream);
    if (a.H == 36 && a.C == 3) return chain::launch16<36, 6>(a, backward, stream);
    if (a.H == 24 && a.C == 2) return chain::launch16<24, 4>(a, backward, stream);
    if (a.H == 12 && a.C == 1) return chain::launch16<12, 2>(a, backward, stream);
    return -2;
  }
  if (a.H == 48 && a.C == 4) return chain::launch<48, 8>(a, backward, stream);
  if (a.H == 36 && a.C == 3) return chain::launch<36, 6>(a, backward, stream);
  if (a.H == 24 && a.C == 2) return chain::launch<24, 4>(a, backward, stream);
  if (a.H == 12 && a.C == 1) return chain::launch<12, 2>(a, backward, stream);
  if (!backward && !a.h_saved) {
    if (a.H == 60 && a.C == 5) return chain::launch_fwd<60, 10>(a, stream);
    if (a.H == 72 && a.C == 6) return chain::launch_fwd<72, 12>(a, stream);
    if (a.H == 84 && a.C == 7) return chain::launch_fwd<84, 14>(a, stream);
    if (a.H == 96 && a.C == 8) return chain::launch_fwd<96, 16>(a, stream);
  }
  return -2;
}

}
```

### lgn-autoencoder_amd/lgn/_native.py

```python
from __future__ import annotations

import ctypes as C
import os
from typing import Optional, Sequence

import torch

_HERE = os.path.dirname(os.path.abspath(__file__))
LIB_PATH = os.environ.get("LGN_AMD_LIB") or os.path.join(_HERE, "_lib", "liblgn_amd.so")
ABI_VERSION = 19
FINALIZE_SCRATCH = 2048
FINALIZE_OPT_SCRATCH = 4096

_lib: Optional[C.CDLL] = None

_vp, _i, _ip = C.c_void_p, C.c_int, C.POINTER(C.c_int)

_SIGNATURES = {
    "lgn_level_fwd_f64": [_i] * 5 + [_vp] * 18,
    "lgn_level_bwd_partial_rows": [_i, _i, _i, _ip, _ip],
    "lgn_level_rad_partial_len": [_i, _i],
    "lgn_level_jet_split": [_i, _i],
    "lgn_cg_product_fwd_f64": [_i] * 8 + [_vp] * 7,
    "lgn_cg_product_bwd_f64": [_i] * 8 + [_vp] * 9,
    "lgn_level_bwd_f64": [_i] * 5 + [_vp] * 24,
    "lgn_reduce_partials_f64": [_vp, _i, _i, _vp, _i, _vp],
    "lgn_radial_finalize_f64": [_vp, _i] + [_vp] * 13,
    "lgn_cgmlp_fwd_f64": [_i] * 5 + [_vp] * 5,
    "lgn_cgmlp_partial_rows": [_i, _i],
    "lgn_cgmlp_bwd_f64": [_i] * 5 + [_vp] * 6 + [_i, _vp],
    "lgn_mixreps_fwd_f64": [_i] * 4 + [_vp] * 4,
    "lgn_chamfer_f64": [_i] * 3 + [_vp] * 2 + [_i] + [_vp] * 4,
    "lgn_mixreps_partial_rows": [_i],
    "lgn_mixreps_bwd_f64": [_i] * 4 + [_vp] * 6,
}


class LocalTables(C.Structure):
    _fields_ = [("n_rows", C.c_int), ("n_out", C.c_int), ("n_w", C.c_int), ("n_terms", C.c_int), ("n_u", C.c_int),
                ("n_x", C.c_int), ("n_units", C.c_int), ("static_kind", C.c_int)] + [
        (name, C.c_void_p) for name in ("row_ptr", "t_type", "t_a", "t_b", "t_coef", "out_dim", "out_nblk", "out_row0", "out_q0",
                                        "out_w0", "u_ptr", "u_row", "u_coef", "x_ptr", "x_row", "x_other", "x_coef")] + [("h_out_w0", C.c_int * 8)]


_tp = C.POINTER(LocalTables)


_POOL_OPS = {"min": 0, "max": 1, "mean": 2, "average": 2}


def pool_code(map_to_latent: str):
    m = map_to_latent.lower()
    if m == "mix":
        return 1 | (3 << 4)
    if "&" in m and "+" in m:
        return None
    avg = "+" in m
    ops = m.split("+") if avg else m.split("&")
    if not 1 <= len(ops) <= 4 or any(o not in _POOL_OPS for o in ops):
        return None
    code = len(ops) | (int(avg) << 3)
    for i, o in enumerate(ops):
        code |= _POOL_OPS[o] << (4 + 2 * i)
    return code


def end_stages_fit(encoder=None, decoder=None, junction: bool = False) -> bool:
    L = lib()
    need = 0
    if encoder is not None:
        code = pool_code(encoder.map_to_latent)
        if code is None:
            return False
        n = encoder.num_input_particles
        ch = encoder.num_channels
        ts, tv = encoder.tau_latent[(0, 0)], encoder.tau_latent[(1, 1)]
        need = max(need, L.lgn_encoder_end_lds_bytes(n, ch[0], max(1, encoder.tau_input_scalars), ch[-1], ts, tv, code))
        if junction and decoder is not None:
            need = max(need, L.lgn_junction_lds_bytes(n, ch[-1], ts, tv, code, decoder.num_channels[0]))
    if decoder is not None:
        ch = decoder.num_channels
        need = max(need, L.lgn_decoder_end_lds_bytes(decoder.num_output_particles, ch[0], decoder.tau_latent_vectors, ch[-1]))
    return 0 <= need <= LDS_LIMIT


def pool_blocks(code: int) -> int:
    if code == 0:
        return 2
    return 1 if (code >> 3) & 1 else code & 7


class NetDesc(C.Structure):
    _fields_ = [("B", C.c_int), ("N", C.c_int), ("n_levels", C.c_int), ("enc_channels", C.c_int * 5),
                ("dec_channels", C.c_int * 5), ("tau_s", C.c_int), ("tau_v", C.c_int), ("mlp_hidden_mul", C.c_int),
                ("mlp_nlin", C.c_int), ("tau_v_in", C.c_int),
                ("enc_tables", _tp * 4), ("dec_tables", _tp * 4),
                ("enc_Q", C.c_int * 5), ("enc_qs", C.c_int * 5), ("enc_qv", C.c_int * 5),
                ("dec_Q", C.c_int * 5), ("dec_qs", C.c_int * 5), ("dec_qv", C.c_int * 5), ("flags", C.c_int),
                ("activation", C.c_int), ("n_in_scalars", C.c_int), ("latent_pool", C.c_int), ("dec_N", C.c_int),
                ("get_real", C.c_int), ("jet_loss_scale", C.c_double)]

    def __init__(self, *a, **kw):
        super().__init__(*a, **kw)
        self.flags = net_flags()


NET_NO_STATIC = 1
_NET_FLAG_ENV = {"LGN_AMD_NO_STATIC": 1, "LGN_AMD_DEC_PAIRWISE": 2, "LGN_AMD_LEVEL_V2": 4, "LGN_AMD_MLP_V1": 8,
                 "LGN_AMD_MOMENTS_V1": 16, "LGN_AMD_BWD_ORDERED": 64, "LGN_AMD_SPLIT_TAIL": 128, "LGN_AMD_DEC_UNFUSED": 256, "LGN_AMD_MOMENTS_SPLIT": 512,
                 "LGN_AMD_MLP_BWD1": 1024}
ACTIVATIONS = {"leakyrelu": 0, "relu": 1, "elu": 2, "sigmoid": 3, "logsigmoid": 4, "atan": 5}


def activation_id(name: str) -> int:
    try:
        return ACTIVATIONS[name.lower()]
    except KeyError:
        raise ValueError(f"Activation function {name} not implemented!") from None


def net_flags() -> int:
    return sum(bit for name, bit in _NET_FLAG_ENV.items() if os.environ.get(name, "") == "1")


class LossDesc(C.Structure):
    _fields_ = [("kind", C.c_int), ("abs_coord", C.c_int), ("polar_coord", C.c_int), ("scale", C.c_double)]


class OptimDesc(C.Structure):
    _fields_ = [("kind", C.c_int), ("l1_lambda", C.c_double), ("l2_lambda", C.c_double), ("lr", C.c_double), ("eps", C.c_double),
                ("beta1", C.c_double), ("beta2", C.c_double), ("alpha", C.c_double), ("momentum", C.c_double)]


OPT_ADAM, OPT_RMSPROP = 0, 1
LOSS_CHAMFER, LOSS_MSE, LOSS_HUNGARIAN = 0, 1, 2
ASSIGN_NMAX = 192
_dp = C.POINTER(NetDesc)
_lp = C.POINTER(LossDesc)
_op = C.POINTER(OptimDesc)
_ll = C.c_longlong
_d = C.c_double
_SIGNATURES.update({
    "lgn_moments_fwd_f64": [_i] * 5 + [_vp] * 12,
    "lgn_moments_bwd_f64": [_i] * 5 + [_vp] * 16,
    "lgn_local_fwd_f64": [_i] * 5 + [_tp] + [_vp] * 5,
    "lgn_local_partial_rows": [_i],
    "lgn_local_fwd_static_f64": [_i] * 4 + [_vp] * 3 + [_ip] + [_vp] * 3 + [_i, _vp],
    "lgn_local_bwd_static_f64": [_i] * 4 + [_vp] * 3 + [_ip] + [_vp] * 8,
    "lgn_local_bwd_f64": [_i] * 5 + [_tp] + [_vp] * 8,
    "lgn_step_param_slots": [_dp, _i],
    "lgn_step_fwd_bwd_f64": [_dp, _vp, _vp, _ll, _vp, _vp, _vp, _vp, _vp, _vp, _vp, _ll, _vp, _vp, _lp, _vp, _vp, _vp],
    "lgn_encoder_fwd_f64": [_dp, _vp, _vp, _vp, _vp, _vp, _vp, _ll, _vp, _vp, _vp],
    "lgn_encoder_bwd_f64": [_dp, _vp, _vp, _ll, _vp, _vp, _vp, _vp, _vp, _ll, _vp, _vp, _vp, _ll, _vp],
    "lgn_decoder_fwd_f64": [_dp, _vp, _vp, _vp, _vp, _ll, _vp, _vp],
    "lgn_decoder_bwd_f64": [_dp, _vp, _vp, _ll, _vp, _vp, _vp, _ll, _vp, _vp, _vp, _ll, _vp],
    "lgn_step_finalize_f64": [_vp, _vp, _ll, _vp, _i, _d, _vp, _vp, _vp, _d, _d, _d, _d, _i, _vp, _vp],
    "lgn_step_train_f64": [_dp, _vp, _vp, _ll, _vp, _vp, _vp, _vp, _vp, _vp, _vp, _ll, _vp, _vp, _i, _d, _vp, _vp, _vp, _d, _d, _d, _d, _i,
                           _vp, _lp, _vp, _vp, _vp],
    "lgn_step_finalize_opt_f64": [_vp, _vp, _ll, _vp, _i, _op, _vp, _vp, _vp, _i, _vp, _vp],
    "lgn_step_train_opt_f64": [_dp, _vp, _vp, _ll, _vp, _vp, _vp, _vp, _vp, _vp, _vp, _ll, _vp, _vp, _i, _op, _vp, _vp, _vp, _i, _vp, _lp,
                               _vp, _vp, _vp],
    "lgn_step_eval_f64": [_dp, _vp, _vp, _vp, _vp, _vp, _vp, _vp, _vp, _ll, _vp, _vp, _vp, _vp, _vp, _lp, _vp, _vp, _vp],
    "lgn_anomaly_scores_f64": [_vp] * 4 + [_i] * 3 + [_vp] * 4,
    "lgn_linear_sum_assignment_f64": [_vp, _i, _i, _vp, _vp, _vp],
    "lgn_hungarian_mse_f64": [_i, _i, _vp, _vp, _i, _i, _i, _d] + [_vp] * 5,
    "lgn_recon_analysis_f64": [_vp, _vp] + [_i] * 4 + [_vp] * 11,
    "lgn_match_rel_err_f64": [_vp] * 6 + [_i, _i] + [_vp] * 5,
    "lgn_histogram_f64": [_vp, _ll, _i, _i, _vp, _ip, _i, _vp, _vp, _vp, _vp, _i, _vp],
    "lgn_stage_batch_f64": [_vp] * 3 + [_i] * 4 + [_d, _i, _i] + [_vp] * 6,
    "lgn_denormalize_f64": [_vp] * 3 + [_i, _i] + [_vp] * 3,
    "lgn_stage_gather_f64": [_vp] * 3 + [_ll, _vp, _ll, _vp] + [_i] * 3 + [_d, _i, _i] + [_vp] * 7,
    "lgn_epoch_collect_f64": [_vp] * 3 + [_ll, _i, _i, C.POINTER(_vp), C.POINTER(_vp), _ip, _vp],
    "lgn_epoch_reset": [_vp] * 4,
    "lgn_roc_auc_f64": [_vp, _ll, _i, _i] + [_vp] * 9 + [_ll, _vp],
    "lgn_emd_f64": [_vp, _vp, _i, _i, _i, _d] + [_vp] * 6 + [_ll, _vp],
    "lgn_emd_relative_f64": [_vp, _vp, _i, _i, _vp, _vp, _vp, _ll, _vp],
    "lgn_emd_debug_max_augmentations": [_ip, _i],
    "lgn_column_stats_f64": [_vp, _ll, _i, _i, _vp, _i, _d, _i] + [_vp] * 5 + [_ll, _vp],
    "lgn_hist_fwhm_f64": [_vp, _i, _vp, _i, _ip, _i, _vp, _vp],
    "lgn_jet_images_f64": [_vp, _vp, _i, _i, _i, _i, _d, _i, _vp, _vp, _vp, _ll, _vp],
    "lgn_transform_jets_f64": [_vp] * 4 + [_i] * 4 + [_vp] * 3,
    "lgn_rep_deviation_f64": [_i] * 3 + [C.POINTER(_vp)] * 3 + [_ip] * 3 + [_vp] * 3 + [_ll, _vp],
})
EPOCH_MAX_COLLECT, EPOCH_BAD_INDEX = 4, 1
NORM_NONE, NORM_COMPONENT_MAX, NORM_OVERALL_MAX, NORM_JET_E = 0, 1, 2, 3


_LL_SIGNATURES = {
    "lgn_step_workspace_doubles": [_dp],
    "lgn_eval_workspace_doubles": [_dp],
    "lgn_net_workspace_doubles": [_dp, _i, _i],
    "lgn_moments_scratch_doubles": [_i, _i, _i, _i],
    "lgn_local_static_packed_doubles": [_i, _i, _i],
    "lgn_encoder_end_lds_bytes": [_i] * 7,
    "lgn_decoder_end_lds_bytes": [_i] * 4,
    "lgn_junction_lds_bytes": [_i] * 6,
    "lgn_assign_loss_lds_bytes": [_i, _i],
    "lgn_roc_workspace_bytes": [_ll, _i],
    "lgn_emd_workspace_bytes": [_i, _i],
    "lgn_emd_lds_bytes": [_i],
    "lgn_column_stats_workspace_bytes": [_ll, _i],
    "lgn_jet_images_workspace_bytes": [_i, _i],
    "lgn_rep_deviation_workspace_bytes": [_i, _i, _i, _ip, _ip, _ip],
}
ROC_TILE, ROC_MAX_COLS = 2048, 65535
ROC_NONFINITE, ROC_SINGLE_CLASS, ROC_BAD_LABEL, ROC_NAN = 1, 2, 4, 8
EMD_NMAX = 191
EMD_INVALID, EMD_EMPTY, EMD_ITER, EMD_INFEASIBLE = 1, 2, 4, 8
HIST_MAX_EDGES, HIST_MAX_COLS = 1025, 16
STATS_TILE, STATS_MAX_COLS, STATS_EMPTY, STATS_NONFINITE = 2048, 16, 1, 2
STAT_NAMES = ("median", "IQR", "first_quartile", "third_quartile", "IDR", "MAD", "mean", "max", "min", "abs_min", "std_dev", "skew",
              "kurtosis", "FWHM", "abs_mean", "abs_mean_within_iqr", "abs_mean_within_idr", "q10", "q90")
STATS_COUNT = len(STAT_NAMES)
JET_IMAGE_MAX_NPIX, JET_IMAGE_PARTS = 64, 512
EQUI_TILE, EQUI_MAX_PARTS = 256, 64
LDS_LIMIT = 160 * 1024
EXPORTED_SYMBOLS = ["lgn_abi_version", "lgn_last_error"] + list(_LL_SIGNATURES) + list(_SIGNATURES)


def lib() -> C.CDLL:
    global _lib
    if _lib is None:
        if not os.path.exists(LIB_PATH):
            raise RuntimeError(
                f"liblgn_amd.so not found at {LIB_PATH}. Build it with `python -c 'import __graft_entry__ as g; "
                "g.build()'` or `make -C lgn-autoencoder_amd/csrc`. There is no CPU fallback.")
        l = C.CDLL(LIB_PATH)
        l.lgn_abi_version.restype = C.c_int
        l.lgn_last_error.restype = C.c_char_p
        got = l.lgn_abi_version()
        if got != ABI_VERSION:
            raise RuntimeError(f"liblgn_amd.so ABI version {got} != expected {ABI_VERSION}; rebuild the library")
        for name, argtypes in _SIGNATURES.items():
            fn = getattr(l, name)
            fn.argtypes = argtypes
            fn.restype = C.c_int
        for name, argtypes in _LL_SIGNATURES.items():
            fn = getattr(l, name)
            fn.argtypes = argtypes
            fn.restype = C.c_longlong
        _lib = l
    return _lib


def last_error() -> str:
    return lib().lgn_last_error().decode()


def _check(rc: int, what: str):
    if rc != 0:
        raise RuntimeError(f"{what} failed (code {rc}): {last_error()}")


def stream_ptr() -> int:
    return torch.cuda.current_stream().cuda_stream


def ptr(t: Optional[torch.Tensor]):
    if t is None:
        return None
    if not t.is_cuda:
        raise RuntimeError("liblgn_amd.so operates on GPU tensors only (got a CPU tensor); there is no CPU fallback")
    if not t.is_contiguous():
        raise RuntimeError("non-contiguous tensor passed to the native library")
    return t.data_ptr()


def f64(t: torch.Tensor) -> torch.Tensor:
    if t.dtype != torch.float64:
        raise RuntimeError(f"the native path is fp64 (reference precision); got {t.dtype}")
    return t.contiguous()



def level_fwd(decoder, s_in, v_in, p, mask, rad, wm0, wm1):
    _, B, N, Cc = s_in.shape
    CO = wm0.shape[1]
    dev, dt = s_in.device, s_in.dtype
    ag0 = torch.empty(2, B, N, 2 * Cc, device=dev, dtype=dt)
    ag1 = torch.empty(2, B, N, 2 * Cc, 4, device=dev, dtype=dt)
    s_out = torch.empty(2, B, N, CO, device=dev, dtype=dt)
    v_out = torch.empty(2, B, N, CO, 4, device=dev, dtype=dt)
    a, b, c, w0, b0, w1, b1 = rad
    rc = lib().lgn_level_fwd_f64(B, N, Cc, CO, int(decoder), ptr(s_in), ptr(v_in), ptr(p), ptr(mask),
                                 ptr(a), ptr(b), ptr(c), ptr(w0), ptr(b0), ptr(w1), ptr(b1), ptr(wm0), ptr(wm1),
                                 ptr(ag0), ptr(ag1), ptr(s_out), ptr(v_out), stream_ptr())
    _check(rc, "lgn_level_fwd_f64")
    return ag0, ag1, s_out, v_out


def reduce_partials(part: torch.Tensor, out: torch.Tensor, accumulate: bool = False):
    rows, n = part.shape
    _check(lib().lgn_reduce_partials_f64(ptr(part), rows, n, ptr(out), int(accumulate), stream_ptr()),
           "lgn_reduce_partials_f64")
    return out


def level_bwd(decoder, s_in, v_in, p, mask, rad, wm0, wm1, ag0, ag1, g_s_out, g_v_out, g_p=None):
    _, B, N, Cc = s_in.shape
    CO = wm0.shape[1]
    dev, dt = s_in.device, s_in.dtype
    L = lib()
    rm, rr = C.c_int(), C.c_int()
    _check(L.lgn_level_bwd_partial_rows(B, N, int(decoder), C.byref(rm), C.byref(rr)), "lgn_level_bwd_partial_rows")
    nmix = 4 * CO * 5 * Cc
    nrad = L.lgn_level_rad_partial_len(Cc, int(decoder))
    part_mix = torch.empty(rm.value, nmix, device=dev, dtype=dt)
    part_rad = torch.empty(rr.value, nrad, device=dev, dtype=dt)
    g_ag = torch.empty(B, N, 20 * Cc, device=dev, dtype=dt)
    g_s_in = torch.empty_like(s_in)
    g_v_in = torch.empty_like(v_in)
    a, b, c, w0, b0, w1, b1 = rad
    rc = L.lgn_level_bwd_f64(B, N, Cc, CO, int(decoder), ptr(s_in), ptr(v_in), ptr(p), ptr(mask),
                             ptr(a), ptr(b), ptr(c), ptr(w0), ptr(b0), ptr(w1), ptr(b1), ptr(wm0), ptr(wm1),
                             ptr(ag0), ptr(ag1), ptr(g_s_out), ptr(g_v_out), ptr(g_ag), ptr(g_s_in), ptr(g_v_in),
                             ptr(g_p), ptr(part_mix), ptr(part_rad), stream_ptr())
    _check(rc, "lgn_level_bwd_f64")
    g_mix = torch.empty(nmix, device=dev, dtype=dt)
    reduce_partials(part_mix, g_mix)
    g_wm0 = g_mix[: nmix // 2].view(2, CO, 5 * Cc)
    g_wm1 = g_mix[nmix // 2:].view(2, CO, 5 * Cc)
    tot = torch.empty(nrad, device=dev, dtype=dt)
    reduce_partials(part_rad, tot)
    if decoder:
        rad_grads = (tot[:Cc], tot[Cc:])
    else:
        g_a, g_b, g_c = (torch.empty_like(x) for x in (a, b, c))
        g_w0, g_b0, g_w1, g_b1 = (torch.empty_like(x) for x in (w0, b0, w1, b1))
        _check(L.lgn_radial_finalize_f64(ptr(tot), Cc, ptr(a), ptr(b), ptr(c), ptr(w0), ptr(w1), ptr(g_a), ptr(g_b),
                                         ptr(g_c), ptr(g_w0), ptr(g_b0), ptr(g_w1), ptr(g_b1), stream_ptr()),
               "lgn_radial_finalize_f64")
        rad_grads = (g_a, g_b, g_c, g_w0, g_b0, g_w1, g_b1)
    return g_s_in, g_v_in, g_wm0, g_wm1, rad_grads


def _ptr_array(ts: Sequence[torch.Tensor]):
    arr = (C.c_void_p * len(ts))()
    for i, t in enumerate(ts):
        arr[i] = ptr(t)
    return arr


def cgmlp_fwd(s_in, ws, bs, act: int = 0):
    _, B, N, Cc = s_in.shape
    H = ws[0].shape[0]
    s_out = torch.empty_like(s_in)
    rc = lib().lgn_cgmlp_fwd_f64(B * N, Cc, H, len(ws), act, _ptr_array(ws), _ptr_array(bs), ptr(s_in), ptr(s_out), stream_ptr())
    _check(rc, "lgn_cgmlp_fwd_f64")
    return s_out


def cgmlp_bwd(s_in, ws, bs, g_out, act: int = 0):
    _, B, N, Cc = s_in.shape
    H = ws[0].shape[0]
    L = lib()
    rows = L.lgn_cgmlp_partial_rows(B * N, H)
    psize = sum(w.numel() + b.numel() for w, b in zip(ws, bs))
    part = torch.empty(rows, psize, device=s_in.device, dtype=s_in.dtype)
    g_in = torch.empty_like(s_in)
    rc = L.lgn_cgmlp_bwd_f64(B * N, Cc, H, len(ws), act, _ptr_array(ws), _ptr_array(bs), ptr(s_in), ptr(g_out), ptr(g_in),
                             ptr(part), psize, stream_ptr())
    _check(rc, "lgn_cgmlp_bwd_f64")
    flat = torch.empty(psize, device=s_in.device, dtype=s_in.dtype)
    reduce_partials(part, flat)
    gws, gbs, off = [], [], 0
    for w, b in zip(ws, bs):
        gws.append(flat[off: off + w.numel()].view_as(w)); off += w.numel()
        gbs.append(flat[off: off + b.numel()].view_as(b)); off += b.numel()
    return g_in, gws, gbs


def chamfer(x, y, jet_features=False):
    x, y = f64(x), f64(y)
    B, Np, M = x.shape[0], x.shape[1], y.shape[1]
    out = torch.empty(B + 4 * B * (Np + M), device=x.device, dtype=x.dtype)
    part, gx, gy = out[:B], out[B:B + 4 * B * Np].view(B, Np, 4), out[B + 4 * B * Np:].view(B, M, 4)
    _check(lib().lgn_chamfer_f64(B, Np, M, ptr(x), ptr(y), int(bool(jet_features)), ptr(part), ptr(gx), ptr(gy), stream_ptr()),
           "lgn_chamfer_f64")
    return part, gx, gy


def hungarian_mse(x, y, kind=LOSS_HUNGARIAN, abs_coord=True, polar_coord=False, scale=None):
    x, y = f64(x), f64(y)
    B, Np = x.shape[0], x.shape[1]
    if scale is None:
        scale = 1.0 / (B * Np * (4 if kind == LOSS_MSE or (abs_coord and not polar_coord) else 3))
    out = torch.empty(B + 4 * B * Np, device=x.device, dtype=x.dtype)
    ints = torch.empty(B * Np + B, device=x.device, dtype=torch.int32)
    part, gx = out[:B], out[B:].view(B, Np, 4)
    assignment, status = ints[:B * Np].view(B, Np), ints[B * Np:]
    _check(lib().lgn_hungarian_mse_f64(B, Np, ptr(x), ptr(y), int(kind), int(bool(abs_coord)), int(bool(polar_coord)), float(scale),
                                       ptr(part), ptr(gx), ptr(assignment), ptr(status), stream_ptr()), "lgn_hungarian_mse_f64")
    return part, gx, assignment, status


def mixreps_fwd(w, x):
    Co, Ci = w.shape[1], w.shape[2]
    d = x.shape[-1]
    rows = x[0].numel() // (Ci * d)
    y = torch.empty(x.shape[:-2] + (Co, d), device=x.device, dtype=x.dtype)
    _check(lib().lgn_mixreps_fwd_f64(rows, Ci, Co, d, ptr(w), ptr(x), ptr(y), stream_ptr()), "lgn_mixreps_fwd_f64")
    return y


def mixreps_bwd(w, x, g_y, need_gx=True):
    Co, Ci = w.shape[1], w.shape[2]
    d = x.shape[-1]
    rows = x[0].numel() // (Ci * d)
    L = lib()
    part = torch.empty(L.lgn_mixreps_partial_rows(rows), 2 * Co * Ci, device=x.device, dtype=x.dtype)
    g_x = torch.empty_like(x) if need_gx else None
    _check(L.lgn_mixreps_bwd_f64(rows, Ci, Co, d, ptr(w), ptr(x), ptr(g_y), ptr(g_x), ptr(part), stream_ptr()),
           "lgn_mixreps_bwd_f64")
    g_w = torch.empty_like(w)
    reduce_partials(part, g_w.view(-1))
    return g_x, g_w



class DeviceTables:

    def __init__(self, tab: dict, device):
        self.meta = tab
        self.tensors = {}
        st = LocalTables()
        st.n_rows, st.n_out, st.n_w = tab["n_rows"], tab["n_out"], tab["n_w"]
        st.n_terms, st.n_u, st.n_x = len(tab["ints"]["t_type"]), len(tab["ints"]["u_row"]), len(tab["ints"]["x_row"])
        st.n_units = 0
        from .plan import static_kind
        st.static_kind = static_kind(tab)
        for i, w0 in enumerate(tab["ints"]["out_w0"][:8]):
            st.h_out_w0[i] = w0
        for name, vals in tab["ints"].items():
            t = torch.tensor(vals if len(vals) else [0], dtype=torch.int32, device=device)
            self.tensors[name] = t
            setattr(st, name, t.data_ptr())
        for name, vals in tab["dbls"].items():
            t = torch.tensor(vals if len(vals) else [0.0], dtype=torch.float64, device=device)
            self.tensors[name] = t
            setattr(st, name, t.data_ptr())
        self.struct = st


def moments_fwd(decoder, X, p, mask, rad, out=None):
    _, B, N, Cc, Q = X.shape
    U = torch.empty(B, N, Cc, Q, 5, 2, device=X.device, dtype=X.dtype) if out is None else out.view(B, N, Cc, Q, 5, 2)
    a, b, c, w0, b0, w1, b1 = rad
    _check(lib().lgn_moments_fwd_f64(B, N, Cc, Q, int(decoder), ptr(X), ptr(p), ptr(mask), ptr(a), ptr(b), ptr(c), ptr(w0),
                                     ptr(b0), ptr(w1), ptr(b1), ptr(U), stream_ptr()), "lgn_moments_fwd_f64")
    return U


def moments_bwd(decoder, X, p, mask, rad, gU, gX, g_p):
    _, B, N, Cc, Q = X.shape
    L = lib()
    nrad = L.lgn_level_rad_partial_len(Cc, int(decoder))
    part = torch.empty(B, nrad, device=X.device, dtype=X.dtype)
    nscr = L.lgn_moments_scratch_doubles(B, N, Cc, int(decoder))
    scratch = torch.empty(nscr, device=X.device, dtype=X.dtype) if nscr > 0 else None
    a, b, c, w0, b0, w1, b1 = rad
    _check(L.lgn_moments_bwd_f64(B, N, Cc, Q, int(decoder), ptr(X), ptr(p), ptr(mask), ptr(a), ptr(b), ptr(c), ptr(w0), ptr(b0),
                                 ptr(w1), ptr(b1), ptr(gU), ptr(gX), ptr(g_p), ptr(part), ptr(scratch), stream_ptr()),
           "lgn_moments_bwd_f64")
    tot = torch.empty(nrad, device=X.device, dtype=X.dtype)
    reduce_partials(part, tot)
    if decoder:
        return (tot[:Cc], tot[Cc:])
    g_a, g_b, g_c = (torch.empty_like(x) for x in (a, b, c))
    g_w0, g_b0, g_w1, g_b1 = (torch.empty_like(x) for x in (w0, b0, w1, b1))
    _check(L.lgn_radial_finalize_f64(ptr(tot), Cc, ptr(a), ptr(b), ptr(c), ptr(w0), ptr(w1), ptr(g_a), ptr(g_b), ptr(g_c),
                                     ptr(g_w0), ptr(g_b0), ptr(g_w1), ptr(g_b1), stream_ptr()), "lgn_radial_finalize_f64")
    return (g_a, g_b, g_c, g_w0, g_b0, g_w1, g_b1)


def local_fwd(tables: DeviceTables, CO, X, U, wcat):
    _, B, N, Cc, Q = X.shape
    Qo = tables.meta["Qout"]
    out = torch.empty(2, B, N, CO, Qo, device=X.device, dtype=X.dtype)
    _check(lib().lgn_local_fwd_f64(B * N, Cc, CO, Q, Qo, C.byref(tables.struct), ptr(X), ptr(U), ptr(wcat), ptr(out), stream_ptr()),
           "lgn_local_fwd_f64")
    return out


def local_bwd(tables: DeviceTables, CO, X, U, wcat, g_out):
    _, B, N, Cc, Q = X.shape
    Qo = tables.meta["Qout"]
    L = lib()
    rows = L.lgn_local_partial_rows(B * N)
    part = torch.empty(rows, wcat.numel(), device=X.device, dtype=X.dtype)
    gU = torch.empty(B, N, Cc, Q, 5, 2, device=X.device, dtype=X.dtype)
    gX = torch.empty_like(X)
    _check(L.lgn_local_bwd_f64(B * N, Cc, CO, Q, Qo, C.byref(tables.struct), ptr(X), ptr(U), ptr(wcat), ptr(g_out), ptr(gU), ptr(gX),
                               ptr(part), stream_ptr()), "lgn_local_bwd_f64")
    g_w = torch.empty_like(wcat)
    reduce_partials(part, g_w)
    return gU, gX, g_w
```

Measured before the change: 1.064 million.

## Compute thin last MLP tile with 4x4x4 f64 MFMA instead of padded 16x16

For hidden widths whose last 16-neuron tile holds at most eight real neurons (H=36, 24, 72), the MLP chain forward and backward kernels now cover that tile with v_mfma_f64_4x4x4 instructions rather than a full 16x16x4 MFMA over zero padding. The item schedule interleaves the thin-tile MFMAs with the full tiles and places the activation/finalize points for the thin tile accordingly. This is meant to cut wasted matrix-core work on padding, at the cost of more complex scheduling and extra, possibly dependent, small MFMAs. An env flag restores the full-tile path, and a standalone probe checks the 4x4x4 layout and cost.

```diff
diff --git a/include/lgn_amd.h b/include/lgn_amd.h
--- a/include/lgn_amd.h
+++ b/include/lgn_amd.h
@@ -149,6 +149,7 @@
 #define LGN_NET_DEC_UNFUSED 256
 #define LGN_NET_MOMENTS_SPLIT 512
 #define LGN_NET_MLP_BWD1 1024
+#define LGN_NET_MLP_FULLTILE 2048
 #define LGN_NET_SPLIT_TAIL 128
 
 #define LGN_LDS_LIMIT (160 * 1024)
diff --git a/lgn-autoencoder_amd/csrc/api_common.cpp b/lgn-autoencoder_amd/csrc/api_common.cpp
--- a/lgn-autoencoder_amd/csrc/api_common.cpp
+++ b/lgn-autoencoder_amd/csrc/api_common.cpp
@@ -16,10 +16,11 @@
   auto on = [](const char* name) { const char* e = getenv(name); return e && e[0] == '1'; };
   return (on("LGN_AMD_DEC_PAIRWISE") ? LVL_DEC_PAIRWISE : 0) | (on("LGN_AMD_LEVEL_V2") ? LVL_LEVEL_V2 : 0) |
          (on("LGN_AMD_MOMENTS_V1") ? LVL_MOMENTS_V1 : 0) | (on("LGN_AMD_MLP_V1") ? LVL_MLP_V1 : 0) | (on("LGN_AMD_BWD_ORDERED") ? LVL_BWD_ORDERED : 0) |
-         (on("LGN_AMD_MOMENTS_SPLIT") ? LVL_MOMENTS_SPLIT : 0) | (on("LGN_AMD_MLP_BWD1") ? LVL_MLP_BWD1 : 0);
+         (on("LGN_AMD_MOMENTS_SPLIT") ? LVL_MOMENTS_SPLIT : 0) | (on("LGN_AMD_MLP_BWD1") ? LVL_MLP_BWD1 : 0) |
+         (on("LGN_AMD_MLP_FULLTILE") ? LVL_MLP_FULLTILE : 0);
 }
 static_assert(LVL_DEC_PAIRWISE == LGN_NET_DEC_PAIRWISE && LVL_LEVEL_V2 == LGN_NET_LEVEL_V2 && LVL_MOMENTS_V1 == LGN_NET_MOMENTS_V1 &&
-                  LVL_MLP_V1 == LGN_NET_MLP_V1 && LVL_MLP_BWD1 == LGN_NET_MLP_BWD1 &&
+                  LVL_MLP_V1 == LGN_NET_MLP_V1 && LVL_MLP_BWD1 == LGN_NET_MLP_BWD1 && LVL_MLP_FULLTILE == LGN_NET_MLP_FULLTILE &&
                   LVL_BWD_ORDERED == LGN_NET_BWD_ORDERED && LVL_MOMENTS_SPLIT == LGN_NET_MOMENTS_SPLIT, "LVL_* and LGN_NET_* are the same bits");
 }
 
diff --git a/lgn-autoencoder_amd/csrc/level.hpp b/lgn-autoencoder_amd/csrc/level.hpp
--- a/lgn-autoencoder_amd/csrc/level.hpp
+++ b/lgn-autoencoder_amd/csrc/level.hpp
@@ -8,6 +8,7 @@
 constexpr int LVL_MLP_V1 = 8;
 constexpr int LVL_MOMENTS_V1 = 16;
 constexpr int LVL_MLP_BWD1 = 1024;
+constexpr int LVL_MLP_FULLTILE = 2048;
 constexpr int LVL_MOMENTS_SPLIT = 512;
 constexpr int LVL_BWD_ORDERED = 64;
 int level_flags_from_env();
diff --git a/lgn-autoencoder_amd/csrc/mlp_chain.hip b/lgn-autoencoder_amd/csrc/mlp_chain.hip
--- a/lgn-autoencoder_amd/csrc/mlp_chain.hip
+++ b/lgn-autoencoder_amd/csrc/mlp_chain.hip
@@ -63,6 +63,8 @@
   static constexpr int NST = NST_;
   static constexpr int NT = (H + 15) / 16, HP = 16 * NT;
   static constexpr int KSH = H / 4;
+  static constexpr int R = H - 16 * (NT - 1), NB = R / 4;
+  static constexpr bool THIN = R <= 8 && NT >= 2;
   static constexpr int KS0 = (D + 3) / 4;
   static constexpr int S = stride2mod4(HP + 1);
   static constexpr int WSIZE = HP * S;
@@ -151,42 +153,77 @@
   issue_image<G, 2>(a, wrA, tid);
 }
 
-template <class G, int KS, int NTI, bool GEN, int DBG = 0, class ExtF>
+template <class G, int KS, bool TH>
+struct Items {
+  static constexpr int NT = G::NT, NB = TH ? G::NB : 0;
+  static constexpr int NF = TH ? NT - 1 : NT;
+  static constexpr int G0 = TH ? KS * (1 + NB) : 0;
+  static constexpr int N = G0 + KS * (TH ? NT - 2 : NT);
+  static_assert(!TH || G::THIN, "a thin last tile");
+  __host__ __device__ static constexpr int tile(int i) {
+    return i >= G0 ? (TH ? 1 : 0) + (i - G0) / KS : i % (1 + NB) == 0 ? 0 : NF + i % (1 + NB) - 1;
+  }
+  __host__ __device__ static constexpr int ks(int i) { return i >= G0 ? (i - G0) % KS : i / (1 + NB); }
+};
+__device__ __forceinline__ double mfma4(double a, double b, double c) { return __builtin_amdgcn_mfma_f64_4x4x4f64(a, b, c, 0, 0, 0); }
+template <class G, int KS, int NTI, bool GEN, bool TH, int DBG = 0, class ExtF>
 __device__ __forceinline__ void layer_fwd(const double* Wc, const v4d (&hin)[NTI], v4d (&hout)[G::NT], int c, int g, int act, ExtF ext) {
-  constexpr int S = G::S, NT = G::NT;
+  using It = Items<G, KS, TH>;
+  constexpr int S = G::S, NT = G::NT, NF = It::NF, NB = It::NB;
   const double* wa = Wc + c * S + g;
+  const double* wt = Wc + (16 * NF + (c & 3)) * S + g;
   const double* wbias = Wc + g * S + G::HP;
   v4d acc[NT];
 #pragma unroll
   for (int r = 0; r < 4; ++r) acc[0][r] = wbias[4 * r * S];
+#pragma unroll
+  for (int q = 0; q < NB; ++q) acc[NT - 1][q] = wbias[(16 * NF + 4 * q) * S];
   if (DBG) STAMP(30);
-  mfma_stream<KS * NT, LOOKAHEAD>(
-      [&](int i) { return wa[16 * (i / KS) * S + 4 * (i % KS)]; },
+  mfma_stream<It::N, LOOKAHEAD>(
+      [&](int i) {
+        const int t = It::tile(i), ks = It::ks(i);
+        return t < NF ? wa[16 * t * S + 4 * ks] : wt[4 * (t - NF) * S + 4 * ks];
+      },
       [&](int i, double av) {
-        const int t = i / KS, ks = i % KS;
-        acc[t] = __builtin_amdgcn_mfma_f64_16x16x4f64(av, hin[ks >> 2][ks & 3], acc[t], 0, 0, 0);
+        const int t = It::tile(i), ks = It::ks(i);
+        if (t < NF) acc[t] = __builtin_amdgcn_mfma_f64_16x16x4f64(av, hin[ks >> 2][ks & 3], acc[t], 0, 0, 0);
+        else acc[NT - 1][t - NF] = mfma4(av, hin[ks >> 2][ks & 3], acc[NT - 1][t - NF]);
       },
       [&](int i) {
-        const int t = i / KS, ks = i % KS;
-        if (ks == 0 && t + 1 < NT) {
-#pragma unroll
-          for (int r = 0; r < 4; ++r) acc[t + 1 < NT ? t + 1 : 0][r] = wbias[(16 * (t + 1) + 4 * r) * S];
+        const int t = It::tile(i), ks = It::ks(i);
+        if (ks == 0 && t + 1 < NF) {
+#pragma unroll
+          for (int r = 0; r < 4; ++r) acc[t + 1 < NF ? t + 1 : 0][r] = wbias[(16 * (t + 1) + 4 * r) * S];
         }
-        constexpr int k1 = KS > 6 ? 5 : KS > 1 ? 1 : 0, k2 = KS > 6 ? 6 : KS > 2 ? 2 : k1;
+        constexpr int k1 = KS > 6 ? 5 : KS > 1 ? 1 : 0, k2 = KS > 6 ? 6 : KS > 2 ? 2 : k1, k3 = k2 + 1 < KS ? k2 + 1 : k2;
 #pragma unroll
         for (int r = 0; r < 4; ++r)
-          if (t > 0 && ks == (r < 2 ? k1 : k2)) {
+          if (t > 0 && t < NF && ks == (r < 2 ? k1 : k2)) {
             double y = act_t<GEN>(acc[t > 0 ? t - 1 : 0][r], act);
             pin(y);
             hout[t > 0 ? t - 1 : 0][r] = y;
+          }
+#pragma unroll
+        for (int q = 0; q < NB; ++q)
+          if (t == 1 && NF > 1 && ks == k3) {
+            double y = act_t<GEN>(acc[NT - 1][q], act);
+            pin(y);
+            hout[NT - 1][q] = y;
           }
         ext(i);
         if (DBG && (i == 0 || i == 1 || i == 2 || i == 11 || i == 12 || i == 23 || i == 34 || i == 35)) STAMP(31 + i);
       });
   if (DBG) STAMP(28);
 #pragma unroll
-  for (int r = 0; r < 4; ++r) hout[NT - 1][r] = act_t<GEN>(acc[NT - 1][r], act);
-  if (DBG) { double z_ = hout[NT - 1][3]; pin(z_); hout[NT - 1][3] = z_; STAMP(29); }
+  for (int r = 0; r < 4; ++r) hout[NF - 1][r] = act_t<GEN>(acc[NF - 1][r], act);
+  if constexpr (TH) {
+#pragma unroll
+    for (int r = 0; r < 4; ++r) {
+      if (r >= NB) hout[NT - 1][r] = 0.0;
+      else if (NF == 1) hout[NT - 1][r] = act_t<GEN>(acc[NT - 1][r], act);
+    }
+  }
+  if (DBG) { double z_ = hout[NF - 1][3]; pin(z_); hout[NF - 1][3] = z_; STAMP(29); }
 }
 template <class G>
 __device__ __forceinline__ v4d layer_out(const double* Wc, const v4d (&hin)[G::NT], int c, int g) {
@@ -200,26 +237,45 @@
                                  [&](int) {});
   return acc;
 }
-template <class G, int KS, int NTO, int NTG, class FinF, class ExtF>
+template <class G, int KS, int NTO, int NTG, bool TH_, class FinF, class ExtF>
 __device__ __forceinline__ void layer_bwd(const double* Wc, const v4d (&gpre)[NTG], v4d (&gin)[NTO], int c, int g, FinF fin, ExtF ext) {
-  constexpr int S = G::S;
+  constexpr bool TH = TH_ && NTO == G::NT;
+  using It = Items<G, KS, TH>;
+  constexpr int S = G::S, NF = TH ? It::NF : NTO, NB = It::NB, N = TH ? It::N : KS * NTO;
   const double* wa = Wc + g * S + c;
+  const double* wt = Wc + g * S + 16 * NF + (c & 3);
 #pragma unroll
   for (int u = 0; u < NTO; ++u) gin[u] = v4d{0, 0, 0, 0};
-  mfma_stream<KS * NTO, LOOKAHEAD>(
-      [&](int i) { return wa[4 * (i % KS) * S + 16 * (i / KS)]; },
+  mfma_stream<N, LOOKAHEAD>(
+      [&](int i) {
+        const int u = It::tile(i), ks = It::ks(i);
+        return u < NF ? wa[4 * ks * S + 16 * u] : wt[4 * ks * S + 4 * (u - NF)];
+      },
       [&](int i, double av) {
-        const int u = i / KS, ks = i % KS;
-        gin[u] = __builtin_amdgcn_mfma_f64_16x16x4f64(av, gpre[ks >> 2][ks & 3], gin[u], 0, 0, 0);
+        const int u = It::tile(i), ks = It::ks(i);
+        if (u < NF) gin[u] = __builtin_amdgcn_mfma_f64_16x16x4f64(av, gpre[ks >> 2][ks & 3], gin[u], 0, 0, 0);
+        else gin[NTO - 1][u - NF] = mfma4(av, gpre[ks >> 2][ks & 3], gin[NTO - 1][u - NF]);
       },
       [&](int i) {
-        const int u = i / KS, ks = i % KS;
-        constexpr int k1 = KS > 6 ? 5 : KS > 1 ? 1 : 0, k2 = KS > 6 ? 6 : KS > 2 ? 2 : k1;
+        const int u = It::tile(i), ks = It::ks(i);
+        constexpr int k1 = KS > 6 ? 5 : KS > 1 ? 1 : 0, k2 = KS > 6 ? 6 : KS > 2 ? 2 : k1, k3 = k2 + 1 < KS ? k2 + 1 : k2;
 #pragma unroll
         for (int r = 0; r < 4; ++r)
-          if (u > 0 && ks == (r < 2 ? k1 : k2)) fin(u > 0 ? u - 1 : 0, r);
+          if (u > 0 && u < NF && ks == (r < 2 ? k1 : k2)) fin(u > 0 ? u - 1 : 0, r);
+#pragma unroll
+        for (int q = 0; q < NB; ++q)
+          if (TH && u == 1 && NF > 1 && ks == k3) fin(NTO - 1, q);
         ext(i);
       });
+}
+template <class G, int NTO, bool TH_, class FinF>
+__device__ __forceinline__ void fin_last(FinF fin, int r) {
+  constexpr bool TH = TH_ && NTO == G::NT;
+  if (!TH) fin(NTO - 1, r);
+  else {
+    fin(NTO - 2, r);
+    if (NTO == 2 && r < G::NB) fin(NTO - 1, r);
+  }
 }
 
 template <class G>
@@ -252,7 +308,7 @@
   }
 }
 
-template <int H, int D, bool GEN, bool SAVE, bool TWO = false>
+template <int H, int D, bool GEN, bool SAVE, bool TWO = false, bool TH = false>
 __global__ __launch_bounds__(TWO ? 512 : 256) void mlp_chain_fwd_kernel(MlpArgs<double> a) {
   using G = Geo<H, D>;
   const int tid = threadIdx.x, lane = tid & 63, wave = __builtin_amdgcn_readfirstlane(tid >> 6);
@@ -284,9 +340,10 @@
   v4d h0[G::NT], h1[G::NT];
   double* hs = SAVE ? saved_ptr<G>(a, wave, lane) : nullptr;
 #define LGN_CHAIN_STEP(Q, HIN, HOUT, KS, NTI)                                                                        \
-  layer_fwd<G, KS, NTI, GEN, (Q == 3)>(Wl + (Q & 1) * G::WSIZE, HIN, HOUT, c, g, a.act, [&](int i) {               \
-    if (!TWO && !LGN_DBG_NOSTAGE) deal<KS * G::NT, stage_pieces<G>()>(i, [&](int j) { stage_piece<G, false, Q>(a, Wl, wrA, wrB, tid, j); });      \
-    if (SAVE && Q > 0) deal<KS * G::NT, 2 * NTI>(i, [&](int j) { save_piece<G>(hs, Q - 1, HIN, j); });              \
+  layer_fwd<G, KS, NTI, GEN, TH, (Q == 3)>(Wl + (Q & 1) * G::WSIZE, HIN, HOUT, c, g, a.act, [&](int i) {           \
+    constexpr int NI = Items<G, KS, TH>::N;                                                                          \
+    if (!TWO && !LGN_DBG_NOSTAGE) deal<NI, stage_pieces<G>()>(i, [&](int j) { stage_piece<G, false, Q>(a, Wl, wrA, wrB, tid, j); });      \
+    if (SAVE && Q > 0) deal<NI, 2 * NTI>(i, [&](int j) { save_piece<G>(hs, Q - 1, HIN, j); });                      \
   });                                                                                                                \
   lds_barrier();                                                                                                     \
   STAMP(2 + Q);
@@ -370,7 +427,7 @@
   return false;
 }
 
-template <int H, int D, bool GEN, bool SAVE>
+template <int H, int D, bool GEN, bool SAVE, bool TH = false>
 __global__ __launch_bounds__(256) void mlp_chain_bwd_kernel(MlpArgs<double> a) {
   using G = Geo<H, D>;
   constexpr int NT = G::NT, NH = G::NH;
@@ -412,8 +469,8 @@
     lds_barrier();
     STAMP(11);
 #define LGN_CHAIN_STEP(Q, HIN, KS, NTI)                                                                              \
-  layer_fwd<G, KS, NTI, GEN>(Wl + (Q & 1) * G::WSIZE, HIN, h[Q], c, g, a.act, [&](int i) {                          \
-    deal<KS * NT, stage_pieces<G>()>(i, [&](int j) { stage_piece<G, true, Q>(a, Wl, wrA, wrB, tid, j); });          \
+  layer_fwd<G, KS, NTI, GEN, TH>(Wl + (Q & 1) * G::WSIZE, HIN, h[Q], c, g, a.act, [&](int i) {                      \
+    deal<Items<G, KS, TH>::N, stage_pieces<G>()>(i, [&](int j) { stage_piece<G, true, Q>(a, Wl, wrA, wrB, tid, j); });  \
   });                                                                                                                \
   lds_barrier();                                                                                                     \
   STAMP(12 + Q);
@@ -425,15 +482,15 @@
     LGN_CHAIN_STEP(5, h[4], G::KSH, NT)
 #undef LGN_CHAIN_STEP
   }
-  v4d gpA[NT], gpB[NT], gin[NT];
+  v4d gpA[NT] = {}, gpB[NT] = {}, gin[NT];
   {
-    constexpr int NI = G::KS0 * NT, NSV = SAVE && NH >= 3 ? saved_pieces<G>() : 0, NPC = 4 + 4 * NT + stage_pieces<G>() + NSV;
+    constexpr int NI = Items<G, G::KS0, TH>::N, NSV = SAVE && NH >= 3 ? saved_pieces<G>() : 0, NPC = 4 + 4 * NT + stage_pieces<G>() + NSV;
     auto fin = [&](int u, int r) {
       double y = gin[u][r] * act_slope_t<GEN>(h[NH - 1][u][r], a.act);
       pin(y);
       gpA[u][r] = y;
     };
-    layer_bwd<G, G::KS0, NT, 1>(Wl + 0 * G::WSIZE, gout, gin, c, g, fin, [&](int i) {
+    layer_bwd<G, G::KS0, NT, 1, TH>(Wl + 0 * G::WSIZE, gout, gin, c, g, fin, [&](int i) {
       deal<NI, NPC>(i, [&](int j) {
         if (j < 4) publish_piece<G, 1>(Gt, gout, wave, c, g, j);
         else if (j < 4 + 4 * NT) publish_piece<G, NT>(Xt, h[NH - 1], wave, c, g, j - 4);
@@ -442,20 +499,20 @@
       });
     });
 #pragma unroll
-    for (int r = 0; r < 4; ++r) fin(NT - 1, r);
+    for (int r = 0; r < 4; ++r) fin_last<G, NT, TH>(fin, r);
     lds_barrier();
     STAMP(18);
   }
 #define LGN_CHAIN_BSTEP(L, GP, GN)                                                                                   \
   {                                                                                                                  \
-    constexpr int q_ = 2 * NH - (L), NI = G::KSH * NT, NSV = SAVE && (L) >= 3 ? saved_pieces<G>() : 0,               \
+    constexpr int q_ = 2 * NH - (L), NI = Items<G, G::KSH, TH>::N, NSV = SAVE && (L) >= 3 ? saved_pieces<G>() : 0,               \
                   NPC = 8 * NT + stage_pieces<G>() + NSV;                                                            \
     auto fin = [&](int u, int r) {                                                                                   \
       double y = gin[u][r] * act_slope_t<GEN>(h[(L) - 1][u][r], a.act);                                              \
       pin(y);                                                                                                        \
       GN[u][r] = y;                                                                                                  \
     };                                                                                                               \
-    layer_bwd<G, G::KSH, NT, NT>(Wl + (q_ & 1) * G::WSIZE, GP, gin, c, g, fin, [&](int i) {                          \
+    layer_bwd<G, G::KSH, NT, NT, TH>(Wl + (q_ & 1) * G::WSIZE, GP, gin, c, g, fin, [&](int i) {                          \
       deal<NI, NPC>(i, [&](int j) {                                                                                  \
         if (j < 4 * NT) publish_piece<G, NT>(Gt + ((L) & 1) * G::TSIZE, GP, wave, c, g, j);                          \
         else if (j < 8 * NT) publish_piece<G, NT>(Xt + ((L) & 1) * G::TSIZE, h[(L) - 1], wave, c, g, j - 4 * NT);    \
@@ -464,8 +521,8 @@
       });                                                                                                            \
     });                                                                                                              \
     auto tail = [&](int i) {                                                                                         \
-      if (i == 1) { fin(NT - 1, 0); fin(NT - 1, 1); }                                                                \
-      if (i == 2) { fin(NT - 1, 2); fin(NT - 1, 3); }                                                                \
+      if (i == 1) { fin_last<G, NT, TH>(fin, 0); fin_last<G, NT, TH>(fin, 1); }                                                                \
+      if (i == 2) { fin_last<G, NT, TH>(fin, 2); fin_last<G, NT, TH>(fin, 3); }                                                                \
     };                                                                                                               \
     if (!dw_layer<G, (L) + 1>(Gt + (((L) + 1) & 1) * G::TSIZE, Xt + (((L) + 1) & 1) * G::TSIZE, part, wave, c, g, tail)) {   \
       tail(1);                                                                                                       \
@@ -482,7 +539,7 @@
 #undef LGN_CHAIN_BSTEP
   {
     v4d gx[1];
-    layer_bwd<G, G::KSH, 1, NT>(Wl + 0 * G::WSIZE, gpB, gx, c, g, [&](int, int) {}, [&](int i) {
+    layer_bwd<G, G::KSH, 1, NT, TH>(Wl + 0 * G::WSIZE, gpB, gx, c, g, [&](int, int) {}, [&](int i) {
       deal<G::KSH, 4 * NT + 4>(i, [&](int j) {
         if (j < 4 * NT) publish_piece<G, NT>(Gt, gpB, wave, c, g, j);
         else publish_piece<G, 1>(Xt, xb, wave, c, g, j - 4 * NT);
@@ -568,7 +625,57 @@
   }
 }
 
-template <int H, int D, bool GEN>
+template <class G, int L, class SideF>
+__device__ __forceinline__ void dw_thin3(const double* Gt, const double* Xt, double* part, int w, int c, int g, SideF side) {
+  static_assert(G::NT == 3 && G::R == 4 && L >= 1 && L < G::NH, "hidden layers of two full tiles and four more neurons");
+  constexpr int SR = G::SR, H = G::H, N = 32, P = 6;
+  const int t = w >> 1, u = w & 1;
+  const bool tr = w >= 2;
+  const double* ga = Gt + (16 * t + c) * SR + g;
+  const double* xb = Xt + (16 * u + c) * SR + g;
+  const double* sa = (tr ? Xt : Gt) + (32 + (c & 3)) * SR + g;
+  const double* sb = (tr ? Gt : Xt) + (16 * u + c) * SR + g;
+  double* pW = part + G::off_w(L);
+  v4d acc = {0, 0, 0, 0};
+  double strip = 0.0, qa[N], qx[N];
+  auto load = [&](int i) {
+    if (i < 16) { qa[i] = ga[4 * i]; qx[i] = xb[4 * i]; }
+    else { qa[i] = sa[4 * (i - 16)]; qx[i] = sb[4 * (i - 16)]; }
+  };
+#pragma unroll
+  for (int i = 0; i < P; ++i) load(i);
+  __builtin_amdgcn_sched_barrier(0);
+#pragma unroll
+  for (int i = 0; i < N; ++i) {
+    if (i + P < N) load(i + P);
+    if (i < 16) acc = __builtin_amdgcn_mfma_f64_16x16x4f64(qa[i], qx[i], acc, 0, 0, 0);
+    else strip = mfma4(qa[i], qx[i], strip);
+    if (i >= 17 && i <= 20) __builtin_nontemporal_store(acc[i - 17], &pW[(16 * t + 4 * (i - 17) + g) * H + 16 * u + c]);
+    side(i);
+    __builtin_amdgcn_sched_barrier(0);
+  }
+  __builtin_nontemporal_store(strip, tr ? &pW[(16 * u + c) * H + 32 + g] : &pW[(32 + g) * H + 16 * u + c]);
+  if (w == 3) {
+    const double* ca = Gt + (32 + (c & 3)) * SR + 16 * (c >> 2) + g;
+    const double* cb = Xt + (32 + (c & 3)) * SR + 16 * (c >> 2) + g;
+    double v = 0.0;
+#pragma unroll
+    for (int sk = 0; sk < 4; ++sk) v = mfma4(ca[4 * sk], cb[4 * sk], v);
+    v += shfl_xor(v, 4);
+    v += shfl_xor(v, 8);
+    if (c < 4) __builtin_nontemporal_store(v, &pW[(32 + g) * H + 32 + c]);
+  } else {
+    double d4[4] = {0.0, 0.0, 0.0, 0.0};
+#pragma unroll
+    for (int sk = 0; sk < 16; ++sk) d4[sk & 3] += w == 1 ? qa[16 + sk] : qa[sk];
+    double dbs = (d4[0] + d4[1]) + (d4[2] + d4[3]);
+    dbs += shfl_xor(dbs, 16);
+    dbs += shfl_xor(dbs, 32);
+    if (g == 0 && (w != 1 || c < 4)) __builtin_nontemporal_store(dbs, &part[G::off_b(L) + (w == 1 ? 32 : 16 * t) + c]);
+  }
+}
+
+template <int H, int D, bool GEN, bool TH = false>
 __global__ __launch_bounds__(512) void mlp_chain_bwd2_kernel(MlpArgs<double> a) {
   using G = Geo<H, D>;
   constexpr int NT = G::NT, NH = G::NH;
@@ -592,18 +699,20 @@
 #define LGN_STAGE_STEP(Q) LGN_STAGE_ALL(Q) lds_barrier();
     LGN_STAGE_STEP(0) LGN_STAGE_STEP(1) LGN_STAGE_STEP(2) LGN_STAGE_STEP(3) LGN_STAGE_STEP(4) LGN_STAGE_STEP(5)
     LGN_STAGE_STEP(6)
-    constexpr bool EVEN = NT == 3;
+    constexpr bool THIN3 = TH && NT == 3 && G::R == 4, EVEN = NT == 3 && !THIN3;
     double* qs = Xt + 2 * G::TSIZE;
 #define LGN_DW_STEP(L)                                                                                               \
   {                                                                                                                  \
     constexpr int q_ = 2 * NH - (L), NS = stage_pieces<G>(), L1 = (L) + 1;                                           \
-    constexpr bool HID = EVEN && L1 >= 1 && L1 < NH;                                                                 \
-    constexpr int NI = HID ? 36 : (L1 == NH || L1 == 0) ? 16 : 16 * NT;                                              \
+    constexpr bool HID = EVEN && L1 >= 1 && L1 < NH, HID3 = THIN3 && L1 >= 1 && L1 < NH;                             \
+    constexpr int NI = HID ? 36 : HID3 ? 32 : (L1 == NH || L1 == 0) ? 16 : 16 * NT;                                  \
     auto side = [&](int i) { deal<NI, NS>(i, [&](int j) { stage_piece<G, true, q_>(a, Wl, wrA, wrB, tid, j); }); };  \
     if constexpr (EVEN && L1 + 1 >= 1 && L1 + 1 < NH) {                                                              \
       if (w4 == 1) dw_quarter_sum<G, (L1 + 1 < NH ? L1 + 1 : 1)>(qs + ((L1 + 1) & 1) * 1024, part, lane, c, g);     \
     }                                                                                                                \
-    if constexpr (HID) {                                                                                             \
+    if constexpr (HID3) {                                                                                            \
+      dw_thin3<G, (HID3 ? L1 : 1)>(Gt + (L1 & 1) * G::TSIZE, Xt + (L1 & 1) * G::TSIZE, part, w4, c, g, side);        \
+    } else if constexpr (HID) {                                                                                      \
       dw_hidden3<G, (HID ? L1 : 1)>(Gt + (L1 & 1) * G::TSIZE, Xt + (L1 & 1) * G::TSIZE, part, qs + (L1 & 1) * 1024, w4, lane, c, g, side); \
     } else if (!dw_layer<G, L1>(Gt + (L1 & 1) * G::TSIZE, Xt + (L1 & 1) * G::TSIZE, part, w4, c, g, side)) {         \
       LGN_STAGE_ALL(q_)                                                                                              \
@@ -636,7 +745,7 @@
   lds_barrier();
   STAMP(11);
 #define LGN_CHAIN_STEP(Q, HIN, KS, NTI)                                                                              \
-  layer_fwd<G, KS, NTI, GEN>(Wl + (Q & 1) * G::WSIZE, HIN, h[Q], c, g, a.act, [&](int) {});                          \
+  layer_fwd<G, KS, NTI, GEN, TH>(Wl + (Q & 1) * G::WSIZE, HIN, h[Q], c, g, a.act, [&](int) {});                          \
   lds_barrier();                                                                                                     \
   STAMP(12 + Q);
   LGN_CHAIN_STEP(0, xb, G::KS0, 1)
@@ -646,41 +755,41 @@
   LGN_CHAIN_STEP(4, h[3], G::KSH, NT)
   LGN_CHAIN_STEP(5, h[4], G::KSH, NT)
 #undef LGN_CHAIN_STEP
-  v4d gpA[NT], gpB[NT], gin[NT];
+  v4d gpA[NT] = {}, gpB[NT] = {}, gin[NT];
   {
-    constexpr int NI = G::KS0 * NT, NPC = 4 + 4 * NT;
+    constexpr int NI = Items<G, G::KS0, TH>::N, NPC = 4 + 4 * NT;
     auto fin = [&](int u, int r) {
       double y = gin[u][r] * act_slope_t<GEN>(h[NH - 1][u][r], a.act);
       pin(y);
       gpA[u][r] = y;
     };
-    layer_bwd<G, G::KS0, NT, 1>(Wl + 0 * G::WSIZE, gout, gin, c, g, fin, [&](int i) {
+    layer_bwd<G, G::KS0, NT, 1, TH>(Wl + 0 * G::WSIZE, gout, gin, c, g, fin, [&](int i) {
       deal<NI, NPC>(i, [&](int j) {
         if (j < 4) publish_piece<G, 1>(Gt, gout, wave, c, g, j);
         else publish_piece<G, NT>(Xt, h[NH - 1], wave, c, g, j - 4);
       });
     });
 #pragma unroll
-    for (int r = 0; r < 4; ++r) fin(NT - 1, r);
+    for (int r = 0; r < 4; ++r) fin_last<G, NT, TH>(fin, r);
     lds_barrier();
     STAMP(18);
   }
 #define LGN_CHAIN_BSTEP(L, GP, GN)                                                                                   \
   {                                                                                                                  \
-    constexpr int q_ = 2 * NH - (L), NI = G::KSH * NT, NPC = 8 * NT;                                                 \
+    constexpr int q_ = 2 * NH - (L), NI = Items<G, G::KSH, TH>::N, NPC = 8 * NT;                                                 \
     auto fin = [&](int u, int r) {                                                                                   \
       double y = gin[u][r] * act_slope_t<GEN>(h[(L) - 1][u][r], a.act);                                              \
       pin(y);                                                                                                        \
       GN[u][r] = y;                                                                                                  \
     };                                                                                                               \
-    layer_bwd<G, G::KSH, NT, NT>(Wl + (q_ & 1) * G::WSIZE, GP, gin, c, g, fin, [&](int i) {                          \
+    layer_bwd<G, G::KSH, NT, NT, TH>(Wl + (q_ & 1) * G::WSIZE, GP, gin, c, g, fin, [&](int i) {                          \
       deal<NI, NPC>(i, [&](int j) {                                                                                  \
         if (j < 4 * NT) publish_piece<G, NT>(Gt + ((L) & 1) * G::TSIZE, GP, wave, c, g, j);                          \
         else publish_piece<G, NT>(Xt + ((L) & 1) * G::TSIZE, h[(L) - 1], wave, c, g, j - 4 * NT);                    \
       });                                                                                                            \
     });                                                                                                              \
     STAMP(56 + (L));                                                                                                 \
-    _Pragma("unroll") for (int r = 0; r < 4; ++r) fin(NT - 1, r);                                                    \
+    _Pragma("unroll") for (int r = 0; r < 4; ++r) fin_last<G, NT, TH>(fin, r);                                                    \
     STAMP(50 + (L));                                                                                                 \
     lds_barrier();                                                                                                   \
     STAMP(12 + q_);                                                                                                  \
@@ -693,7 +802,7 @@
 #undef LGN_CHAIN_BSTEP
   {
     v4d gx[1];
-    layer_bwd<G, G::KSH, 1, NT>(Wl + 0 * G::WSIZE, gpB, gx, c, g, [&](int, int) {}, [&](int i) {
+    layer_bwd<G, G::KSH, 1, NT, TH>(Wl + 0 * G::WSIZE, gpB, gx, c, g, [&](int, int) {}, [&](int i) {
       deal<G::KSH, 4 * NT + 4>(i, [&](int j) {
         if (j < 4 * NT) publish_piece<G, NT>(Gt, gpB, wave, c, g, j);
         else publish_piece<G, 1>(Xt, xb, wave, c, g, j - 4 * NT);
@@ -739,7 +848,7 @@
   v4d h0[G::NT], h1[G::NT];
   double* hs = SAVE ? saved_ptr16<G>(a, lane) : nullptr;
 #define LGN_CHAIN_STEP(Q, HIN, HOUT, KS, NTI)                                                                        \
-  layer_fwd<G, KS, NTI, GEN>(Wl + (Q & 1) * G::WSIZE, HIN, HOUT, c, g, a.act, [&](int i) {                          \
+  layer_fwd<G, KS, NTI, GEN, false>(Wl + (Q & 1) * G::WSIZE, HIN, HOUT, c, g, a.act, [&](int i) {                          \
     if (SAVE && Q > 0) deal<KS * G::NT, 2 * NTI>(i, [&](int j) { save_piece<G>(hs, Q - 1, HIN, j); });              \
   });                                                                                                                \
   lds_barrier();
@@ -871,7 +980,7 @@
   } else {
     lds_barrier();
 #define LGN_CHAIN_STEP(Q, HIN, KS, NTI)                                                                              \
-  layer_fwd<G, KS, NTI, GEN>(Wl + (Q & 1) * G::WSIZE, HIN, h[Q], c, g, a.act, [&](int) {});                          \
+  layer_fwd<G, KS, NTI, GEN, false>(Wl + (Q & 1) * G::WSIZE, HIN, h[Q], c, g, a.act, [&](int) {});                          \
   lds_barrier();
     LGN_CHAIN_STEP(0, xb, G::KS0, 1)
     LGN_CHAIN_STEP(1, h[0], G::KSH, NT)
@@ -889,7 +998,7 @@
       pin(y);
       gpA[u][r] = y;
     };
-    layer_bwd<G, G::KS0, NT, 1>(Wl + 0 * G::WSIZE, gout, gin, c, g, fin, [&](int i) {
+    layer_bwd<G, G::KS0, NT, 1, false>(Wl + 0 * G::WSIZE, gout, gin, c, g, fin, [&](int i) {
       deal<NI, NPC>(i, [&](int j) {
         if (j < 4) publish_piece<G, 1>(Gt, gout, 0, c, g, j);
         else if (j < 4 + 4 * NT) publish_piece<G, NT>(Xt, h[NH - 1], 0, c, g, j - 4);
@@ -908,7 +1017,7 @@
       pin(y);                                                                                                        \
       GN[u][r] = y;                                                                                                  \
     };                                                                                                               \
-    layer_bwd<G, G::KSH, NT, NT>(Wl + (q_ & 1) * G::WSIZE, GP, gin, c, g, fin, [&](int i) {                          \
+    layer_bwd<G, G::KSH, NT, NT, false>(Wl + (q_ & 1) * G::WSIZE, GP, gin, c, g, fin, [&](int i) {                          \
       deal<NI, NPC>(i, [&](int j) {                                                                                  \
         if (j < 4 * NT) publish_piece<G, NT>(Gt + ((L) & 1) * G::TSIZE, GP, 0, c, g, j);                             \
         else if (j < 8 * NT) publish_piece<G, NT>(Xt + ((L) & 1) * G::TSIZE, h[(L) - 1], 0, c, g, j - 4 * NT);       \
@@ -926,7 +1035,7 @@
 #undef LGN_CHAIN_BSTEP
   {
     v4d gx[1];
-    layer_bwd<G, G::KSH, 1, NT>(Wl + 0 * G::WSIZE, gpB, gx, c, g, [&](int, int) {}, [&](int i) {
+    layer_bwd<G, G::KSH, 1, NT, false>(Wl + 0 * G::WSIZE, gpB, gx, c, g, [&](int, int) {}, [&](int i) {
       deal<G::KSH, 4 * NT + 4>(i, [&](int j) {
         if (j < 4 * NT) publish_piece<G, NT>(Gt, gpB, 0, c, g, j);
         else publish_piece<G, 1>(Xt, xb, 0, c, g, j - 4 * NT);
@@ -1248,20 +1357,20 @@
   return 0;
 }
 
-template <int H, int D>
+template <int H, int D, bool TH>
 static int launch_fwd(const MlpArgs<double>& a, hipStream_t stream) {
   using G = Geo<H, D>;
   static_assert(G::fwd_bytes() <= 160 * 1024, "LDS budget");
   const bool two = !(a.flags & LVL_MLP_BWD1);
-  auto kern = two ? (a.act == 0 ? mlp_chain_fwd_kernel<H, D, false, false, true> : mlp_chain_fwd_kernel<H, D, true, false, true>)
-                  : (a.act == 0 ? mlp_chain_fwd_kernel<H, D, false, false> : mlp_chain_fwd_kernel<H, D, true, false>);
+  auto kern = two ? (a.act == 0 ? mlp_chain_fwd_kernel<H, D, false, false, true, TH> : mlp_chain_fwd_kernel<H, D, true, false, true, TH>)
+                  : (a.act == 0 ? mlp_chain_fwd_kernel<H, D, false, false, false, TH> : mlp_chain_fwd_kernel<H, D, true, false, false, TH>);
   (void)hipFuncSetAttribute(reinterpret_cast<const void*>(kern), hipFuncAttributeMaxDynamicSharedMemorySize, (int)G::fwd_bytes());
   hipLaunchKernelGGL(kern, dim3(cdiv(a.M, 64)), dim3(two ? 512 : 256), G::fwd_bytes(), stream, a);
   LGN_CHECK_LAUNCH();
   return 0;
 }
 
-template <int H, int D>
+template <int H, int D, bool TH>
 static int launch(const MlpArgs<double>& a, bool backward, hipStream_t stream) {
   using G = Geo<H, D>;
   const int nblk = cdiv(a.M, 64);
@@ -1271,27 +1380,33 @@
   LGN_CHECK_ARG(!a.h_saved || a.h_rows >= nblk * 64, "cgmlp: the saved-activation buffer has %d rows per layer, %d rows need %d",
                 a.h_rows, a.M, nblk * 64);
   if (backward && !a.h_saved && !(a.flags & LVL_MLP_BWD1)) {
-    auto k2 = a.act == 0 ? mlp_chain_bwd2_kernel<H, D, false> : mlp_chain_bwd2_kernel<H, D, true>;
+    auto k2 = a.act == 0 ? mlp_chain_bwd2_kernel<H, D, false, TH> : mlp_chain_bwd2_kernel<H, D, true, TH>;
+    const size_t smem2 = smem - (TH && G::NT == 3 && G::R == 4 ? sizeof(double) * 2 * 1024 : 0);
+    if (smem2 > 64 * 1024) (void)hipFuncSetAttribute(reinterpret_cast<const void*>(k2), hipFuncAttributeMaxDynamicSharedMemorySize, (int)smem2);
+    hipLaunchKernelGGL(k2, dim3(nblk), dim3(512), smem2, stream, a);
+    LGN_CHECK_LAUNCH();
+    return 0;
+  }
+  if (!backward && !a.h_saved && !(a.flags & LVL_MLP_BWD1)) {
+    auto k2 = a.act == 0 ? mlp_chain_fwd_kernel<H, D, false, false, true, TH> : mlp_chain_fwd_kernel<H, D, true, false, true, TH>;
     if (smem > 64 * 1024) (void)hipFuncSetAttribute(reinterpret_cast<const void*>(k2), hipFuncAttributeMaxDynamicSharedMemorySize, (int)smem);
     hipLaunchKernelGGL(k2, dim3(nblk), dim3(512), smem, stream, a);
     LGN_CHECK_LAUNCH();
     return 0;
   }
-  if (!backward && !a.h_saved && !(a.flags & LVL_MLP_BWD1)) {
-    auto k2 = a.act == 0 ? mlp_chain_fwd_kernel<H, D, false, false, true> : mlp_chain_fwd_kernel<H, D, true, false, true>;
-    if (smem > 64 * 1024) (void)hipFuncSetAttribute(reinterpret_cast<const void*>(k2), hipFuncAttributeMaxDynamicSharedMemorySize, (int)smem);
-    hipLaunchKernelGGL(k2, dim3(nblk), dim3(512), smem, stream, a);
-    LGN_CHECK_LAUNCH();
-    return 0;
-  }
-  auto kern = a.h_saved ? (a.act == 0 ? (backward ? mlp_chain_bwd_kernel<H, D, false, true> : mlp_chain_fwd_kernel<H, D, false, true>)
-                                      : (backward ? mlp_chain_bwd_kernel<H, D, true, true> : mlp_chain_fwd_kernel<H, D, true, true>))
-                        : (a.act == 0 ? (backward ? mlp_chain_bwd_kernel<H, D, false, false> : mlp_chain_fwd_kernel<H, D, false, false>)
-                                      : (backward ? mlp_chain_bwd_kernel<H, D, true, false> : mlp_chain_fwd_kernel<H, D, true, false>));
+  auto kern = a.h_saved ? (a.act == 0 ? (backward ? mlp_chain_bwd_kernel<H, D, false, true, TH> : mlp_chain_fwd_kernel<H, D, false, true, false, TH>)
+                                      : (backward ? mlp_chain_bwd_kernel<H, D, true, true, TH> : mlp_chain_fwd_kernel<H, D, true, true, false, TH>))
+                        : (a.act == 0 ? (backward ? mlp_chain_bwd_kernel<H, D, false, false, TH> : mlp_chain_fwd_kernel<H, D, false, false, false, TH>)
+                                      : (backward ? mlp_chain_bwd_kernel<H, D, true, false, TH> : mlp_chain_fwd_kernel<H, D, true, false, false, TH>));
   if (smem > 64 * 1024) (void)hipFuncSetAttribute(reinterpret_cast<const void*>(kern), hipFuncAttributeMaxDynamicSharedMemorySize, (int)smem);
   hipLaunchKernelGGL(kern, dim3(nblk), dim3(256), smem, stream, a);
   LGN_CHECK_LAUNCH();
   return 0;
+}
+template <int H, int D>
+static int launch_thin(const MlpArgs<double>& a, bool backward, hipStream_t stream) {
+  static_assert(Geo<H, D>::THIN, "a last tile of at most eight neurons");
+  return (a.flags & LVL_MLP_FULLTILE) ? launch<H, D, false>(a, backward, stream) : launch<H, D, true>(a, backward, stream);
 }
 
 }
@@ -1309,15 +1424,15 @@
     if (a.H == 12 && a.C == 1) return chain::launch16<12, 2>(a, backward, stream);
     return -2;
   }
-  if (a.H == 48 && a.C == 4) return chain::launch<48, 8>(a, backward, stream);
-  if (a.H == 36 && a.C == 3) return chain::launch<36, 6>(a, backward, stream);
-  if (a.H == 24 && a.C == 2) return chain::launch<24, 4>(a, backward, stream);
-  if (a.H == 12 && a.C == 1) return chain::launch<12, 2>(a, backward, stream);
+  if (a.H == 48 && a.C == 4) return chain::launch<48, 8, false>(a, backward, stream);
+  if (a.H == 36 && a.C == 3) return chain::launch_thin<36, 6>(a, backward, stream);
+  if (a.H == 24 && a.C == 2) return chain::launch_thin<24, 4>(a, backward, stream);
+  if (a.H == 12 && a.C == 1) return chain::launch<12, 2, false>(a, backward, stream);
   if (!backward && !a.h_saved) {
-    if (a.H == 60 && a.C == 5) return chain::launch_fwd<60, 10>(a, stream);
-    if (a.H == 72 && a.C == 6) return chain::launch_fwd<72, 12>(a, stream);
-    if (a.H == 84 && a.C == 7) return chain::launch_fwd<84, 14>(a, stream);
-    if (a.H == 96 && a.C == 8) return chain::launch_fwd<96, 16>(a, stream);
+    if (a.H == 60 && a.C == 5) return chain::launch_fwd<60, 10, false>(a, stream);
+    if (a.H == 72 && a.C == 6) return (a.flags & LVL_MLP_FULLTILE) ? chain::launch_fwd<72, 12, false>(a, stream) : chain::launch_fwd<72, 12, true>(a, stream);
+    if (a.H == 84 && a.C == 7) return chain::launch_fwd<84, 14, false>(a, stream);
+    if (a.H == 96 && a.C == 8) return chain::launch_fwd<96, 16, false>(a, stream);
   }
   return -2;
 }
diff --git a/lgn-autoencoder_amd/csrc/probes/mfma4_probe.hip b/lgn-autoencoder_amd/csrc/probes/mfma4_probe.hip
--- /dev/null
+++ b/lgn-autoencoder_amd/csrc/probes/mfma4_probe.hip
@@ -0,0 +1,111 @@
+#include <hip/hip_runtime.h>
+#include <cstdio>
+typedef double v4d __attribute__((ext_vector_type(4)));
+
+__global__ void layout(double* out) {
+  const int lane = threadIdx.x;
+  for (int la = 0; la < 64; ++la) {
+    const double a = lane == la ? 1.0 : 0.0, b = 1.0 + lane;
+    out[la * 64 + lane] = __builtin_amdgcn_mfma_f64_4x4x4f64(a, b, 0.0, 0, 0, 0);
+  }
+}
+
+constexpr int GROUPS = 24;
+template <int VAR>
+__global__ __launch_bounds__(256) void cost(double* out, long long* cyc, int rounds) {
+  const int lane = threadIdx.x & 63;
+  double a0 = 1e-3 * lane, a1 = 2e-3 * lane, a2 = 1e-3 * (lane & 3), b = 1.0 + 1e-3 * lane;
+  v4d f0 = {0, 0, 0, 0}, f1 = {0, 0, 0, 0};
+  double t0 = 0, t1 = 0, t2 = 0, t3 = 0;
+  const long long c0 = clock64();
+  for (int r = 0; r < rounds; ++r) {
+#pragma unroll
+    for (int s = 0; s < GROUPS; ++s) {
+      if (VAR == 0) t0 = __builtin_amdgcn_mfma_f64_4x4x4f64(a2, b, t0, 0, 0, 0);
+      if (VAR == 1) {
+        if (s & 1) t1 = __builtin_amdgcn_mfma_f64_4x4x4f64(a2, b, t1, 0, 0, 0);
+        else t0 = __builtin_amdgcn_mfma_f64_4x4x4f64(a2, b, t0, 0, 0, 0);
+      }
+      if (VAR == 2) {
+        if ((s & 3) == 0) t0 = __builtin_amdgcn_mfma_f64_4x4x4f64(a2, b, t0, 0, 0, 0);
+        if ((s & 3) == 1) t1 = __builtin_amdgcn_mfma_f64_4x4x4f64(a2, b, t1, 0, 0, 0);
+        if ((s & 3) == 2) t2 = __builtin_amdgcn_mfma_f64_4x4x4f64(a2, b, t2, 0, 0, 0);
+        if ((s & 3) == 3) t3 = __builtin_amdgcn_mfma_f64_4x4x4f64(a2, b, t3, 0, 0, 0);
+      }
+      if (VAR == 3) {
+        if (s & 1) f1 = __builtin_amdgcn_mfma_f64_16x16x4f64(a1, b, f1, 0, 0, 0);
+        else f0 = __builtin_amdgcn_mfma_f64_16x16x4f64(a0, b, f0, 0, 0, 0);
+      }
+      if (VAR == 4) {
+        f0 = __builtin_amdgcn_mfma_f64_16x16x4f64(a0, b, f0, 0, 0, 0);
+        f1 = __builtin_amdgcn_mfma_f64_16x16x4f64(a1, b, f1, 0, 0, 0);
+        t0 = __builtin_amdgcn_mfma_f64_4x4x4f64(a2, b, t0, 0, 0, 0);
+      }
+      if (VAR == 5) {
+        f0 = __builtin_amdgcn_mfma_f64_16x16x4f64(a0, b, f0, 0, 0, 0);
+        t0 = __builtin_amdgcn_mfma_f64_4x4x4f64(a2, b, t0, 0, 0, 0);
+      }
+      if (VAR == 6) {
+        f0 = __builtin_amdgcn_mfma_f64_16x16x4f64(a0, b, f0, 0, 0, 0);
+        t0 = __builtin_amdgcn_mfma_f64_4x4x4f64(a2, b, t0, 0, 0, 0);
+        t1 = __builtin_amdgcn_mfma_f64_4x4x4f64(a2, b, t1, 0, 0, 0);
+      }
+      __builtin_amdgcn_sched_barrier(0);
+    }
+    b = fmax(b, 1e-30 * (f0[0] + f1[1] + t0 + t1 + t2 + t3));
+  }
+  const long long c1 = clock64();
+  out[blockIdx.x * blockDim.x + threadIdx.x] = f0[0] + f0[3] + f1[1] + t0 + t1 + t2 + t3 + b;
+  if (threadIdx.x == 0 && blockIdx.x == 0) cyc[0] = c1 - c0;
+}
+
+template <int VAR>
+static double run(const char* what, int full, int thin, double* out, long long* cyc) {
+  const int rounds = 2000;
+  long long h = 0;
+  for (int pass = 0; pass < 2; ++pass) {
+    hipLaunchKernelGGL(cost<VAR>, dim3(256), dim3(256), 0, 0, out, cyc, rounds);
+    hipDeviceSynchronize();
+    hipMemcpy(&h, cyc, 8, hipMemcpyDeviceToHost);
+  }
+  const double per_group = (double)h / ((double)rounds * GROUPS);
+  printf("variant %d: %-58s %7.1f cycles per group of %d full + %d thin\n", VAR, what, per_group, full, thin);
+  return per_group;
+}
+
+int main() {
+  double* out; long long* cyc;
+  hipMalloc(&out, 1 << 24); hipMalloc(&cyc, 8);
+  static double h[64 * 64];
+  hipLaunchKernelGGL(layout, dim3(1), dim3(64), 0, 0, out);
+  hipDeviceSynchronize();
+  hipMemcpy(h, out, sizeof(h), hipMemcpyDeviceToHost);
+  printf("layout of v_mfma_f64_4x4x4_4b_f64: A = one-hot at lane la, B = 1 + lane; 'd<-b' = D lane d received B lane b\n");
+  int bad = 0;
+  for (int la = 0; la < 64; ++la) {
+    printf("  A lane %2d:", la);
+    int n = 0;
+    for (int d = 0; d < 64; ++d) {
+      const double v = h[la * 64 + d];
+      if (v != 0.0) { printf(" %d<-%d", d, (int)v - 1); ++n; }
+      const int i = la & 3, blk = (la >> 2) & 3, k = la >> 4;
+      const double want = ((d >> 4) == i && ((d >> 2) & 3) == blk) ? 1.0 + 16 * k + 4 * blk + (d & 3) : 0.0;
+      if (v != want) ++bad;
+    }
+    printf("%s\n", n == 4 ? "" : "   (not four lanes)");
+  }
+  printf("assumed mapping  A: i = l & 3, b = (l >> 2) & 3, k = l >> 4   B: j = l & 3, b = (l >> 2) & 3, k = l >> 4   D: j = l & 3, b = (l >> 2) & 3, i = l >> 4\n");
+  printf("  -> %s (%d of 4096 entries differ)\n", bad == 0 ? "CONFIRMED" : "NOT what the instruction does", bad);
+  printf("cost, one wave per SIMD, 256 workgroups of 256 threads, %d groups per round:\n", GROUPS);
+  const double c0 = run<0>("thin, one accumulator (dependent chain)", 0, 1, out, cyc);
+  const double c1 = run<1>("thin, two alternating accumulators", 0, 1, out, cyc);
+  const double c2 = run<2>("thin, four accumulators", 0, 1, out, cyc);
+  const double c3 = run<3>("full 16x16x4, two alternating accumulators", 1, 0, out, cyc);
+  const double c4 = run<4>("full, full, thin sharing B (1 : 2, one thin accumulator)", 2, 1, out, cyc);
+  const double c5 = run<5>("full, thin sharing B (1 : 1, one thin accumulator)", 1, 1, out, cyc);
+  const double c6 = run<6>("full, thin, thin sharing B (two thin accumulators)", 1, 2, out, cyc);
+  printf("cycles per thin instruction: chain %.1f | two accumulators %.1f | four %.1f | full instruction %.1f\n", c0, c1, c2, c3);
+  printf("interleaved cost of a thin instruction (group - full instructions): 1:2 %.1f | 1:1 %.1f | 1 full + 2 thin %.1f each\n",
+         c4 - 2 * c3, c5 - c3, (c6 - c3) / 2);
+  return 0;
+}
diff --git a/lgn-autoencoder_amd/lgn/_native.py b/lgn-autoencoder_amd/lgn/_native.py
--- a/lgn-autoencoder_amd/lgn/_native.py
+++ b/lgn-autoencoder_amd/lgn/_native.py
@@ -108,7 +108,7 @@
 NET_NO_STATIC = 1
 _NET_FLAG_ENV = {"LGN_AMD_NO_STATIC": 1, "LGN_AMD_DEC_PAIRWISE": 2, "LGN_AMD_LEVEL_V2": 4, "LGN_AMD_MLP_V1": 8,
                  "LGN_AMD_MOMENTS_V1": 16, "LGN_AMD_BWD_ORDERED": 64, "LGN_AMD_SPLIT_TAIL": 128, "LGN_AMD_DEC_UNFUSED": 256, "LGN_AMD_MOMENTS_SPLIT": 512,
-                 "LGN_AMD_MLP_BWD1": 1024}
+                 "LGN_AMD_MLP_BWD1": 1024, "LGN_AMD_MLP_FULLTILE": 2048}
 ACTIVATIONS = {"leakyrelu": 0, "relu": 1, "elu": 2, "sigmoid": 3, "logsigmoid": 4, "atan": 5}
 
 
```

Result: faster. 1.092 million (median of 6 runs) (+2.7%).
